# JettHuang/jet-pbrt

Hardware: AMD Instinct MI355X
Metric: Msamples/sec (whole node) + per-pixel L2 vs CPU ref, cornell_box 1024spp (higher is better)
Workload: dtype f32

## Files before the change

jet-pbrt_amd/csrc/jp_device.h:

```cpp
#pragma once
#include <hip/hip_runtime.h>
#include <stdint.h>
#include "jetpbrt_amd.h"
#include "jp_counter_rng.h"

#define JP_BLOCK 256
#define JP_STACK_DEPTH 32

namespace jp
{
struct V3 { float x, y, z; };
__device__ __forceinline__ V3 mk(float x, float y, float z) { V3 v; v.x = x; v.y = y; v.z = z; return v; }
__device__ __forceinline__ V3 operator+(V3 a, V3 b) { return mk(a.x + b.x, a.y + b.y, a.z + b.z); }
__device__ __forceinline__ V3 operator-(V3 a, V3 b) { return mk(a.x - b.x, a.y - b.y, a.z - b.z); }
__device__ __forceinline__ V3 operator-(V3 a) { return mk(-a.x, -a.y, -a.z); }
__device__ __forceinline__ V3 operator*(V3 a, float s) { return mk(a.x * s, a.y * s, a.z * s); }
__device__ __forceinline__ V3 operator*(float s, V3 a) { return mk(a.x * s, a.y * s, a.z * s); }
__device__ __forceinline__ V3 operator/(V3 a, float s) { return mk(a.x / s, a.y / s, a.z / s); }
__device__ __forceinline__ V3 cmul(V3 a, V3 b) { return mk(a.x * b.x, a.y * b.y, a.z * b.z); }
__device__ __forceinline__ V3 cdiv(V3 a, V3 b) { return mk(a.x / b.x, a.y / b.y, a.z / b.z); }
__device__ __forceinline__ V3 splat(float v) { return mk(v, v, v); }
__device__ __forceinline__ V3 csqrt(V3 a) { return mk(sqrtf(a.x), sqrtf(a.y), sqrtf(a.z)); }
__device__ __forceinline__ float dot(V3 a, V3 b) { return a.x * b.x + a.y * b.y + a.z * b.z; }
__device__ __forceinline__ float len2(V3 a) { return a.x * a.x + a.y * a.y + a.z * a.z; }
__device__ __forceinline__ float len(V3 a) { return sqrtf(len2(a)); }
__device__ __forceinline__ V3 normalize(V3 a) { return a / len(a); }
__device__ __forceinline__ V3 cross(V3 a, V3 v) { return mk(a.y * v.z - a.z * v.y, a.z * v.x - a.x * v.z, a.x * v.y - a.y * v.x); }
__device__ __forceinline__ float absdot(V3 a, V3 b) { return fabsf(dot(a, b)); }
__device__ __forceinline__ bool isblack(V3 c) { return c.x == 0.f && c.y == 0.f && c.z == 0.f; }
__device__ __forceinline__ float smin(float a, float b) { return (b < a) ? b : a; }
__device__ __forceinline__ float smax(float a, float b) { return (a < b) ? b : a; }
__device__ __forceinline__ float maxcomp(V3 c) { float m = (c.y < c.z) ? c.z : c.y; return (c.x < m) ? m : c.x; }
__device__ __forceinline__ float clampf(float v, float lo, float hi) { if (v < lo) return lo; else if (v > hi) return hi; else return v; }
__device__ __forceinline__ V3 xyz(float4 v) { return mk(v.x, v.y, v.z); }

#define JP_PI      3.14159274101257324219f
#define JP_INF     __int_as_float(0x7f800000)

struct SceneView
{
	const float4* nodes; int n_nodes;
	const float4* prims; const int4* meta; int n_prims;
	const float4* mats;
	const int* mat_type; int n_mats;
	const float4* lights;
	int n_lights;
	const float4* shade_tab;
	float3 env_sum;
	int n_env;
	float world_radius;
	JpCamera cam;
	const float4* flat; int n_flat;
	const uint4* wide; int n_wide;
	const uint4* q4; int n_q4;
	const float4* refbox; float cert_pad, cert_pad_eye;
};

__device__ __forceinline__ bool tri_hit(V3 p0, V3 p1, V3 p2, V3 n, V3 o, V3 d, float tmin, float& tmax)
{
	const V3 oa = p0 - o;
	const float distance = dot(n, oa) / dot(n, d);
	if (!((distance > tmin) && (distance < tmax))) return false;
	const V3 ob = p1 - o, oc = p2 - o;
	const V3 v0 = cross(oc, ob), v1 = cross(ob, oa), v2 = cross(oa, oc);
	const float v0d = dot(v0, d), v1d = dot(v1, d), v2d = dot(v2, d);
	if (((v0d < 0) && (v1d < 0) && (v2d < 0)) || ((v0d >= 0) && (v1d >= 0) && (v2d >= 0))) { tmax = distance; return true; }
	return false;
}
__device__ __forceinline__ bool rect_hit(V3 p0, V3 p1, V3 p2, V3 p3, V3 n, V3 o, V3 d, float tmin, float& tmax)
{
	const V3 oa = p0 - o;
	const float distance = dot(n, oa) / dot(n, d);
	if (!((distance > tmin) && (distance < tmax))) return false;
	const V3 ob = p1 - o, oc = p2 - o, od = p3 - o;
	const V3 v0 = cross(oc, ob), v1 = cross(ob, oa), v2 = cross(oa, od), v3 = cross(od, oc);
	const float v0d = dot(v0, d), v1d = dot(v1, d), v2d = dot(v2, d), v3d = dot(v3, d);
	if (((v0d < 0) && (v1d < 0) && (v2d < 0) && (v3d < 0)) || ((v0d >= 0) && (v1d >= 0) && (v2d >= 0) && (v3d >= 0))) { tmax = distance; return true; }
	return false;
}
__device__ __forceinline__ bool sph_hit(V3 c, float r, V3 o, V3 d, float tmin, float& tmax)
{
	V3 oc = o - c;
	float a = len2(d);
	float half_b = dot(oc, d);
	float cc = len2(oc) - r * r;
	float disc = half_b * half_b - a * cc;
	if (disc > 0.0f)
	{
		float root = sqrtf(disc);
		float time;
		float root1 = (-half_b - root) / a;
		if (root1 < tmax && root1 > tmin) time = root1;
		else
		{
			float root2 = (-half_b + root) / a;
			if (root2 < tmax && root2 > tmin) time = root2;
			else return false;
		}
		tmax = time;
		return true;
	}
	return false;
}

__device__ __forceinline__ bool disk_hit(V3 c, float r, V3 n, V3 o, V3 d, float tmin, float& tmax)
{
	const float dn = dot(d, n);
	if (fabsf(dn - 0.f) <= 1.1920928955078125e-07f * smax(1.f, smax(fabsf(dn), fabsf(0.f)))) return false;
	const V3 op = c - o;
	const float distance = dot(n, op) / dot(n, d);
	if ((distance > tmin) && (distance < tmax))
	{
		const V3 hp = o + distance * d;
		if (len(c - hp) <= r) { tmax = distance; return true; }
	}
	return false;
}

template <int kS, typename PrimPtr>
__device__ __forceinline__ bool prim_hit(PrimPtr prims, int pi, V3 o, V3 d, float tmin, float& tmax)
{
	const float4 g0 = prims[kS * pi + 0], g1 = prims[kS * pi + 1], g2 = prims[kS * pi + 2], g3 = prims[kS * pi + 3];
	const int type = __float_as_int(g3.w);
	if (type == JP_SHAPE_TRIANGLE) return tri_hit(xyz(g0), xyz(g1), xyz(g2), xyz(g3), o, d, tmin, tmax);
	if (type == JP_SHAPE_SPHERE) return sph_hit(xyz(g0), g0.w, o, d, tmin, tmax);
	if (type == JP_SHAPE_DISK) return disk_hit(xyz(g0), g0.w, xyz(g1), o, d, tmin, tmax);
	return rect_hit(xyz(g0), xyz(g1), xyz(g2), mk(g0.w, g1.w, g2.w), xyz(g3), o, d, tmin, tmax);
}

template <bool kAnyHit, int kS, typename NodePtr, typename PrimPtr>
__device__ __forceinline__ int traverse(NodePtr nodes, PrimPtr prims, V3 o, V3 d, float tmin, float& tmax, int* stack)
{
	const float ix = 1.0f / d.x, iy = 1.0f / d.y, iz = 1.0f / d.z;
	int hit = -1, sp = 0, cur = 0;
	for (;;)
	{
		bool alive = true;
		while (cur >= 0)
		{
			const float4 n0 = nodes[kS * cur + 0], n1 = nodes[kS * cur + 1], n2 = nodes[kS * cur + 2], n3 = nodes[kS * cur + 3];
			const float lx0 = (n0.x - o.x) * ix, lx1 = (n0.w - o.x) * ix;
			const float ly0 = (n0.y - o.y) * iy, ly1 = (n1.x - o.y) * iy;
			const float lz0 = (n0.z - o.z) * iz, lz1 = (n1.y - o.z) * iz;
			const float ln = fmaxf(fmaxf(fminf(lx0, lx1), fminf(ly0, ly1)), fmaxf(fminf(lz0, lz1), tmin));
			const float lf = fminf(fminf(fmaxf(lx0, lx1), fmaxf(ly0, ly1)), fminf(fmaxf(lz0, lz1), tmax));
			const float rx0 = (n1.z - o.x) * ix, rx1 = (n2.y - o.x) * ix;
			const float ry0 = (n1.w - o.y) * iy, ry1 = (n2.z - o.y) * iy;
			const float rz0 = (n2.x - o.z) * iz, rz1 = (n2.w - o.z) * iz;
			const float rn = fmaxf(fmaxf(fminf(rx0, rx1), fminf(ry0, ry1)), fmaxf(fminf(rz0, rz1), tmin));
			const float rf = fminf(fminf(fmaxf(rx0, rx1), fmaxf(ry0, ry1)), fminf(fmaxf(rz0, rz1), tmax));
			const bool hl = ln <= lf * 1.000002f, hr = rn <= rf * 1.000002f;
			const int cl = __float_as_int(n3.x), cr = __float_as_int(n3.y);
			if (hl && hr)
			{
				const bool leftFirst = kAnyHit ? true : (ln <= rn);
				cur = leftFirst ? cl : cr;
				stack[sp * JP_BLOCK] = leftFirst ? cr : cl; sp++;
			}
			else if (hl) cur = cl;
			else if (hr) cur = cr;
			else if (sp > 0) { sp--; cur = stack[sp * JP_BLOCK]; }
			else { alive = false; break; }
		}
		if (!alive) break;
		const int e = -cur - 1, first = e >> 4, count = (e & 15) + 1;
		for (int k = 0; k < count; k++)
			if (prim_hit<kS>(prims, first + k, o, d, tmin, tmax)) { hit = first + k; if (kAnyHit) return hit; }
		if (sp > 0) { sp--; cur = stack[sp * JP_BLOCK]; } else break;
	}
	return hit;
}

__device__ __forceinline__ bool ref_box_exact(float4 n0, float4 n1, V3 o, V3 d, float tmin, float tmax)
{
	float bt0 = tmin, bt1 = tmax;
	{
		const float lo = (n0.x - o.x) / d.x, hi = (n1.x - o.x) / d.x;
		bt0 = smax(smin(lo, hi), bt0); bt1 = smin(smax(lo, hi), bt1);
		if (bt1 <= bt0) return false;
	}
	{
		const float lo = (n0.y - o.y) / d.y, hi = (n1.y - o.y) / d.y;
		bt0 = smax(smin(lo, hi), bt0); bt1 = smin(smax(lo, hi), bt1);
		if (bt1 <= bt0) return false;
	}
	{
		const float lo = (n0.z - o.z) / d.z, hi = (n1.z - o.z) / d.z;
		bt0 = smax(smin(lo, hi), bt0); bt1 = smin(smax(lo, hi), bt1);
		if (bt1 <= bt0) return false;
	}
	return true;
}
__device__ __forceinline__ bool ref_box(float4 n0, float4 n1, V3 o, V3 d, V3 rd, float tmin, float tmax)
{
	const float x0 = (n0.x - o.x) * rd.x, x1 = (n1.x - o.x) * rd.x;
	const float y0 = (n0.y - o.y) * rd.y, y1 = (n1.y - o.y) * rd.y;
	const float z0 = (n0.z - o.z) * rd.z, z1 = (n1.z - o.z) * rd.z;
	const float t0 = fmaxf(fmaxf(fminf(x0, x1), fminf(y0, y1)), fmaxf(fminf(z0, z1), tmin));
	const float t1 = fminf(fminf(fmaxf(x0, x1), fmaxf(y0, y1)), fminf(fmaxf(z0, z1), tmax));
	const float s = x0 + x1 + y0 + y1 + z0 + z1;
	const float margin = 2e-6f * (fabsf(t0) + fabsf(t1));
	const float gap = t1 - t0;
	if (fabsf(s) <= 3.0e38f && fabsf(gap) > margin) return gap > 0.f;
	return ref_box_exact(n0, n1, o, d, tmin, tmax);
}

template <bool kAnyHit>
__device__ __forceinline__ int traverse_ref(const float4* __restrict__ nodes, const float4* __restrict__ prims, V3 o, V3 d, float tmin, float& tmax, int* stack)
{
	const V3 rd = mk(__builtin_amdgcn_rcpf(d.x), __builtin_amdgcn_rcpf(d.y), __builtin_amdgcn_rcpf(d.z));
	int hit = -1, sp = 0, cur = 0;
	for (;;)
	{
		const float4 n0 = nodes[2 * cur], n1 = nodes[2 * cur + 1];
		const bool ok = ref_box(n0, n1, o, d, rd, tmin, tmax);
		const int left = __float_as_int(n0.w), right = __float_as_int(n1.w);
		if (ok && left >= 0) { stack[sp * JP_BLOCK] = right; sp++; cur = left; continue; }
		if (ok)
		{
			const int first = -left - 1;
			for (int k = 0; k < right; k++)
				if (prim_hit<4>(prims, first + k, o, d, tmin, tmax)) { hit = first + k; if (kAnyHit) return hit; }
		}
		if (sp == 0) break;
		sp--; cur = stack[sp * JP_BLOCK];
	}
	return hit;
}

typedef const __attribute__((address_space(4))) float* ConstFPtr;
typedef unsigned long long u64;
template <bool k64> struct FlatMask { typedef unsigned int type; };
template <> struct FlatMask<true> { typedef u64 type; };
template <bool k64> __device__ __forceinline__ int mask_count(typename FlatMask<k64>::type m) { return k64 ? __popcll((u64)m) : __popc((unsigned int)m); }

template <bool k64>
__device__ __forceinline__ typename FlatMask<k64>::type flat_boxes(const float4* flat_g, int n_flat, V3 o, V3 d, float tmin, float tmax)
{
	typedef typename FlatMask<k64>::type M;
	ConstFPtr flat = (ConstFPtr)flat_g;
	const float ix = __builtin_amdgcn_rcpf(d.x), iy = __builtin_amdgcn_rcpf(d.y), iz = __builtin_amdgcn_rcpf(d.z);
	M mask = 0;
	#define JP_FLAT_BOX(i) \
	{ \
		const float x0 = (flat[8 * (i) + 0] - o.x) * ix, x1 = (flat[8 * (i) + 4] - o.x) * ix; \
		const float y0 = (flat[8 * (i) + 1] - o.y) * iy, y1 = (flat[8 * (i) + 5] - o.y) * iy; \
		const float z0 = (flat[8 * (i) + 2] - o.z) * iz, z1 = (flat[8 * (i) + 6] - o.z) * iz; \
		const float tn = fmaxf(fmaxf(fminf(x0, x1), fminf(y0, y1)), fmaxf(fminf(z0, z1), tmin)); \
		const float tf = fminf(fminf(fmaxf(x0, x1), fmaxf(y0, y1)), fminf(fmaxf(z0, z1), tmax)); \
		M bits = (M)__float_as_uint(flat[8 * (i) + 3]); \
		if (k64) bits |= (M)((u64)__float_as_uint(flat[8 * (i) + 7]) << 32); \
		if (tn <= tf * 1.000002f) mask |= bits; \
	}
	int i0 = 0;
	for (; i0 + 4 <= n_flat; i0 += 4)
	{
		#pragma unroll
		for (int u = 0; u < 4; u++) JP_FLAT_BOX(i0 + u)
	}
	for (; i0 < n_flat; i0++) JP_FLAT_BOX(i0)
	#undef JP_FLAT_BOX
	return mask;
}

template <bool kAnyHit, bool k64, int kS, typename PrimPtr>
__device__ __forceinline__ int flat_prims(typename FlatMask<k64>::type mask, PrimPtr prims, V3 o, V3 d, float tmin, float& tmax)
{
	int hit = -1;
#ifdef JP_DBG_FLAT_P1ONLY
	mask = mask == (typename FlatMask<k64>::type)0x12345677u ? 1u : 0u;
#endif
	while (mask)
	{
		const int p = (k64 ? __ffsll((unsigned long long)mask) : __ffs((int)mask)) - 1;
		mask &= mask - 1;
		if (prim_hit<kS>(prims, p, o, d, tmin, tmax)) { hit = p; if (kAnyHit) return hit; }
	}
	return hit;
}

template <bool kAnyHit, int kS, typename PrimPtr>
__device__ __forceinline__ int traverse_flat(const float4* flat_g, int n_flat, int n_prims, PrimPtr prims, V3 o, V3 d, float tmin, float& tmax)
{
	if (n_prims > 32) return flat_prims<kAnyHit, true, kS>(flat_boxes<true>(flat_g, n_flat, o, d, tmin, tmax), prims, o, d, tmin, tmax);
	return flat_prims<kAnyHit, false, kS>(flat_boxes<false>(flat_g, n_flat, o, d, tmin, tmax), prims, o, d, tmin, tmax);
}

template <bool kAnyHit, typename PrimPtr>
__device__ __forceinline__ int traverse_wide(const uint4* __restrict__ wide, PrimPtr prims, V3 o, V3 d, float tmin, float& tmax, unsigned int* stack)
{
	const float ix = 1.0f / d.x, iy = 1.0f / d.y, iz = 1.0f / d.z;
	const unsigned int octinv = 7u - ((d.x < 0 ? 1u : 0u) | (d.y < 0 ? 2u : 0u) | (d.z < 0 ? 4u : 0u));
	unsigned int ngx = 0, ngy = 0x80000000u;
	int hit = -1, sp = 0;
	for (;;)
	{
		unsigned int tgx = 0, tgy = 0;
		if (ngy > 0x00ffffffu)
		{
			const unsigned int bit = 31u - (unsigned int)__clz((int)ngy);
			ngy &= ~(1u << bit);
			if (ngy > 0x00ffffffu) { stack[(2 * sp) * JP_BLOCK] = ngx; stack[(2 * sp + 1) * JP_BLOCK] = ngy; sp++; }
			const unsigned int slot = (bit - 24u) ^ octinv;
			const unsigned int rel = (unsigned int)__popc(ngy & 0xffu & ~(0xffffffffu << slot));
			const unsigned int idx = ngx + rel;
			const uint4 q0 = wide[5 * idx + 0], q1 = wide[5 * idx + 1], q2 = wide[5 * idx + 2], q3 = wide[5 * idx + 3], q4 = wide[5 * idx + 4];
			const float sx = __uint_as_float(((q0.w & 0xffu) ) << 23), sy = __uint_as_float(((q0.w >> 8) & 0xffu) << 23), sz = __uint_as_float(((q0.w >> 16) & 0xffu) << 23);
			const float px = __uint_as_float(q0.x) - o.x, py = __uint_as_float(q0.y) - o.y, pz = __uint_as_float(q0.z) - o.z;
			unsigned int hm = 0;
			#pragma unroll
			for (int i = 0; i < 8; i++)
			{
				const int sh = 8 * (i & 3);
				const unsigned int m = ((i < 4 ? q1.z : q1.w) >> sh) & 0xffu;
				const float lx = (float)(((i < 4 ? q2.x : q2.y) >> sh) & 0xffu), ly = (float)(((i < 4 ? q2.z : q2.w) >> sh) & 0xffu), lz = (float)(((i < 4 ? q3.x : q3.y) >> sh) & 0xffu);
				const float hx = (float)(((i < 4 ? q3.z : q3.w) >> sh) & 0xffu), hy = (float)(((i < 4 ? q4.x : q4.y) >> sh) & 0xffu), hz = (float)(((i < 4 ? q4.z : q4.w) >> sh) & 0xffu);
				const float x0 = fmaf(lx, sx, px) * ix, x1 = fmaf(hx, sx, px) * ix;
				const float y0 = fmaf(ly, sy, py) * iy, y1 = fmaf(hy, sy, py) * iy;
				const float z0 = fmaf(lz, sz, pz) * iz, z1 = fmaf(hz, sz, pz) * iz;
				const float tn = fmaxf(fmaxf(fminf(x0, x1), fminf(y0, y1)), fmaxf(fminf(z0, z1), tmin));
				const float tf = fminf(fminf(fmaxf(x0, x1), fmaxf(y0, y1)), fminf(fmaxf(z0, z1), tmax));
				if (m != 0u && tn <= tf * 1.000002f)
				{
					const bool inner = (m & 0x18u) == 0x18u;
					const unsigned int bits = inner ? 1u : (m >> 5), at = inner ? 24u + ((m & 7u) ^ octinv) : (m & 31u);
					hm |= bits << at;
				}
			}
			ngx = q1.x; ngy = (hm & 0xff000000u) | (q0.w >> 24);
			tgx = q1.y; tgy = hm & 0x00ffffffu;
		}
		while (tgy)
		{
			const int j = __ffs((int)tgy) - 1;
			tgy &= tgy - 1;
			if (prim_hit<4>(prims, (int)tgx + j, o, d, tmin, tmax)) { hit = (int)tgx + j; if (kAnyHit) return hit; }
		}
		if (ngy <= 0x00ffffffu)
		{
			if (sp == 0) break;
			sp--; ngx = stack[(2 * sp) * JP_BLOCK]; ngy = stack[(2 * sp + 1) * JP_BLOCK];
		}
	}
	return hit;
}

struct WalkStack
{
	int* lds; int* spill; int cap; unsigned int stride;
	__device__ __forceinline__ void put(int at, int v) const { if (at < cap) lds[at * JP_BLOCK] = v; else spill[(size_t)(at - cap) * stride] = v; }
	__device__ __forceinline__ int get(int at) const { return at < cap ? lds[at * JP_BLOCK] : spill[(size_t)(at - cap) * stride]; }
};

template <int kMode> struct Walker;

template <> struct Walker<0>
{
	V3 o, d; float ix, iy, iz, tmin, tmax; int cur, sp, hit; bool done;
	__device__ __forceinline__ void start(V3 o_, V3 d_, float tmin_, float tmax_)
	{ o = o_; d = d_; ix = 1.0f / d.x; iy = 1.0f / d.y; iz = 1.0f / d.z; tmin = tmin_; tmax = tmax_; cur = 0; sp = 0; hit = -1; done = false; }
	__device__ __forceinline__ bool heavy() const { return cur < 0; }
	template <bool kAnyHit> __device__ __forceinline__ void step(const SceneView& sc, const WalkStack& stack)
	{
		if (cur >= 0)
		{
			const float4* __restrict__ nodes = sc.nodes;
			const float4 n0 = nodes[4 * cur + 0], n1 = nodes[4 * cur + 1], n2 = nodes[4 * cur + 2], n3 = nodes[4 * cur + 3];
			const float lx0 = (n0.x - o.x) * ix, lx1 = (n0.w - o.x) * ix;
			const float ly0 = (n0.y - o.y) * iy, ly1 = (n1.x - o.y) * iy;
			const float lz0 = (n0.z - o.z) * iz, lz1 = (n1.y - o.z) * iz;
			const float ln = fmaxf(fmaxf(fminf(lx0, lx1), fminf(ly0, ly1)), fmaxf(fminf(lz0, lz1), tmin));
			const float lf = fminf(fminf(fmaxf(lx0, lx1), fmaxf(ly0, ly1)), fminf(fmaxf(lz0, lz1), tmax));
			const float rx0 = (n1.z - o.x) * ix, rx1 = (n2.y - o.x) * ix;
			const float ry0 = (n1.w - o.y) * iy, ry1 = (n2.z - o.y) * iy;
			const float rz0 = (n2.x - o.z) * iz, rz1 = (n2.w - o.z) * iz;
			const float rn = fmaxf(fmaxf(fminf(rx0, rx1), fminf(ry0, ry1)), fmaxf(fminf(rz0, rz1), tmin));
			const float rf = fminf(fminf(fmaxf(rx0, rx1), fmaxf(ry0, ry1)), fminf(fmaxf(rz0, rz1), tmax));
			const bool hl = ln <= lf * 1.000002f, hr = rn <= rf * 1.000002f;
			const int cl = __float_as_int(n3.x), cr = __float_as_int(n3.y);
			if (hl && hr)
			{
				const bool leftFirst = kAnyHit ? true : (ln <= rn);
				cur = leftFirst ? cl : cr;
				stack.put(sp, leftFirst ? cr : cl); sp++;
			}
			else if (hl) cur = cl;
			else if (hr) cur = cr;
			else if (sp > 0) { sp--; cur = stack.get(sp); }
			else done = true;
		}
		else
		{
			const int e = -cur - 1, first = e >> 4, count = (e & 15) + 1;
			for (int k = 0; k < count; k++)
				if (prim_hit<4>(sc.prims, first + k, o, d, tmin, tmax)) { hit = first + k; if (kAnyHit) { done = true; return; } }
			if (sp > 0) { sp--; cur = stack.get(sp); } else done = true;
		}
	}
};

template <> struct Walker<5>
{
	V3 o, d, rd; float tmin, tmax; int cur, sp, hit, lfirst, lcount, lk; bool done;
	__device__ __forceinline__ void start(V3 o_, V3 d_, float tmin_, float tmax_)
	{ o = o_; d = d_; rd = mk(__builtin_amdgcn_rcpf(d.x), __builtin_amdgcn_rcpf(d.y), __builtin_amdgcn_rcpf(d.z)); tmin = tmin_; tmax = tmax_; cur = 0; sp = 0; hit = -1; lcount = 0; lk = 0; lfirst = 0; done = false; }
	__device__ __forceinline__ bool heavy() const { return lcount > 0; }
	template <bool kAnyHit> __device__ __forceinline__ void step(const SceneView& sc, const WalkStack& stack)
	{
		if (lcount > 0)
		{
			if (prim_hit<4>(sc.prims, lfirst + lk, o, d, tmin, tmax)) { hit = lfirst + lk; if (kAnyHit) { done = true; return; } }
			if (++lk < lcount) return;
			lcount = 0; lk = 0;
		}
		else
		{
			const float4* __restrict__ nodes = sc.nodes;
			const float4 n0 = nodes[2 * cur], n1 = nodes[2 * cur + 1];
			const bool ok = ref_box(n0, n1, o, d, rd, tmin, tmax);
			const int left = __float_as_int(n0.w), right = __float_as_int(n1.w);
			if (ok && left >= 0) { stack.put(sp, right); sp++; cur = left; return; }
			if (ok && right > 0) { lfirst = -left - 1; lcount = right; lk = 0; return; }
		}
		if (sp == 0) { done = true; return; }
		sp--; cur = stack.get(sp);
	}
};

template <> struct Walker<3>
{
	V3 o, d; float ix, iy, iz, tmin, tmax; unsigned int ngx, ngy, tgx, tgy, octinv; int sp, hit; bool done;
	__device__ __forceinline__ void start(V3 o_, V3 d_, float tmin_, float tmax_)
	{
		o = o_; d = d_; ix = 1.0f / d.x; iy = 1.0f / d.y; iz = 1.0f / d.z; tmin = tmin_; tmax = tmax_;
		octinv = 7u - ((d.x < 0 ? 1u : 0u) | (d.y < 0 ? 2u : 0u) | (d.z < 0 ? 4u : 0u));
		ngx = 0; ngy = 0x80000000u; tgx = tgy = 0; sp = 0; hit = -1; done = false;
	}
	__device__ __forceinline__ bool heavy() const { return tgy == 0u && ngy > 0x00ffffffu; }
// ... 187 lines not shown
```

jet-pbrt_amd/csrc/jp_kernels.hip:

```cpp
#include "jp_common.h"
#include "jp_tex.h"
#include "jp_xbsdf.h"

#include <cstdio>
#include <cstring>
#include <string>
#include <vector>
#include <algorithm>
#include <cmath>
#include <mutex>
#include <thread>
#include "jp_devmem.h"
#include "jp_lbvh.h"
#include "jp_ploc.h"

__global__ void __launch_bounds__(JP_BLOCK) k_raygen(SceneView sc, Queues q, RenderConst rc, DevCounters* cnt)
{
	const unsigned int total = (unsigned int)rc.npix * rc.sbatch;
	const unsigned int nchunks = (total + JP_BLOCK - 1) / JP_BLOCK;
	const unsigned int G = gridDim.x, b = blockIdx.x;
	if (b == 0 && threadIdx.x == 0) { cnt->n_queue[0] = total; cnt->n_queue[1] = 0; cnt->n_shadow = 0; }
	unsigned int filled = 0;
	const unsigned int K = (nchunks + G - 1) / G, npb = (unsigned int)rc.npix / JP_BLOCK;
	for (unsigned int k = 0, j0 = 0; k < K; k++, j0 += JP_BLOCK)
	{
		unsigned int c;
		if (rc.compact) { const unsigned int qi = b * K + k; if (qi >= nchunks) break; const unsigned int pb = qi / (unsigned int)rc.sbatch, sl = qi - pb * (unsigned int)rc.sbatch; c = sl * npb + pb; }
		else { c = b + k * G; if (c >= nchunks) break; }
		const unsigned int slot = c * JP_BLOCK + threadIdx.x;
		if (slot < total)
		{
			const unsigned int i = b * q.R + j0 + threadIdx.x;
			const int pix = slot % rc.npix, s = rc.s0 + slot / rc.npix;
			int x, y; pixel_of(rc, pix, x, y);
			const uint32_t key = jp_rng_key(rc.seed, (uint32_t)x, (uint32_t)y, (uint32_t)s);
			const float fx = (float)x + rngf(rc, key, 0), fy = (float)y + rngf(rc, key, 1);
			const V3 front = mk(sc.cam.front[0], sc.cam.front[1], sc.cam.front[2]);
			const V3 right = mk(sc.cam.right[0], sc.cam.right[1], sc.cam.right[2]);
			const V3 up = mk(sc.cam.up[0], sc.cam.up[1], sc.cam.up[2]);
			V3 dir = front + right * (fx / sc.cam.res_x - 0.5f) + up * (0.5f - fy / sc.cam.res_y);
			dir = normalize(dir);
			q.ray_o[0][i] = make_float4(sc.cam.pos[0], sc.cam.pos[1], sc.cam.pos[2], __int_as_float((int)slot));
			q.ray_d[0][i] = make_float4(dir.x, dir.y, dir.z, __int_as_float(MK_FLAGS(0, 0, 2)));
			q.beta[0][i] = make_float4(1.f, 1.f, 1.f, __int_as_float((int)key));
			q.lacc[slot] = make_float4(0.f, 0.f, 0.f, 0.f);
		}
		const unsigned int left = total - c * JP_BLOCK;
		filled += left < JP_BLOCK ? left : JP_BLOCK;
	}
	if (threadIdx.x == 0) q.blk_q[0][b] = filled;
}


#if defined(JP_SHADE_TIMING) || defined(JP_TRAV_TIMING)
__device__ unsigned long long g_shade_t[16];
#define JP_TSX(i) do { const unsigned long long t_ = __builtin_amdgcn_s_memtime(); t_acc[i] += t_ - t_last; t_last = t_; } while (0)
#endif
#ifdef JP_SHADE_TIMING
#define JP_TS(i) JP_TSX(i)
#else
#define JP_TS(i) do { } while (0)
#endif
#ifdef JP_TRAV_TIMING
#define JP_TT(i) JP_TSX(i)
#else
#define JP_TT(i) do { } while (0)
#endif
template <int kMode>
struct SceneAccess;
template <> struct SceneAccess<0>
{
	const float4 *nodes, *prims; int* stack; int depth;
	__device__ __forceinline__ SceneAccess(const SceneView& sc, int depth_) : nodes(sc.nodes), prims(sc.prims), stack((int*)s_dyn + threadIdx.x), depth(depth_) {}
	template <bool kAnyHit> __device__ __forceinline__ int trace(const SceneView&, V3 o, V3 d, float tmin, float& tmax) const
	{ return traverse<kAnyHit, 4>(nodes, prims, o, d, tmin, tmax, stack); }
};
template <> struct SceneAccess<1>
{
	float4 *nodes, *prims; int* stack; int depth;
	__device__ __forceinline__ SceneAccess(const SceneView& sc, int depth_) : depth(depth_)
	{
		stack = (int*)s_dyn + threadIdx.x;
		nodes = s_dyn + (depth * JP_BLOCK) / 4;
		prims = nodes + 5 * sc.n_nodes;
		for (int i = threadIdx.x; i < 4 * sc.n_nodes; i += JP_BLOCK) nodes[5 * (i >> 2) + (i & 3)] = sc.nodes[i];
		for (int i = threadIdx.x; i < 4 * sc.n_prims; i += JP_BLOCK) prims[5 * (i >> 2) + (i & 3)] = sc.prims[i];
		__syncthreads();
	}
	template <bool kAnyHit> __device__ __forceinline__ int trace(const SceneView&, V3 o, V3 d, float tmin, float& tmax) const
	{ return traverse<kAnyHit, 5>(nodes, prims, o, d, tmin, tmax, stack); }
};
template <> struct SceneAccess<2>
{
	float4* prims;
	__device__ __forceinline__ SceneAccess(const SceneView& sc, int)
	{
		prims = s_dyn;
		for (int i = threadIdx.x; i < 4 * sc.n_prims; i += JP_BLOCK) prims[5 * (i >> 2) + (i & 3)] = sc.prims[i];
		__syncthreads();
	}
	template <bool kAnyHit> __device__ __forceinline__ int trace(const SceneView& sc, V3 o, V3 d, float tmin, float& tmax) const
	{ return traverse_flat<kAnyHit, 5>(sc.flat, sc.n_flat, sc.n_prims, prims, o, d, tmin, tmax); }
};

template <> struct SceneAccess<3>
{
	const float4* prims; unsigned int* stack;
	__device__ __forceinline__ SceneAccess(const SceneView& sc, int) : prims(sc.prims), stack((unsigned int*)s_dyn + threadIdx.x) {}
	template <bool kAnyHit> __device__ __forceinline__ int trace(const SceneView& sc, V3 o, V3 d, float tmin, float& tmax) const
	{ return traverse_wide<kAnyHit>(sc.wide, prims, o, d, tmin, tmax, stack); }
};

template <> struct SceneAccess<4>
{
	WalkStack stack;
	__device__ __forceinline__ SceneAccess(const SceneView&, int depth) { stack.lds = (int*)s_dyn + threadIdx.x; stack.spill = nullptr; stack.cap = depth - 1; stack.stride = 0; }
	template <bool kAnyHit> __device__ __forceinline__ int trace(const SceneView& sc, V3 o, V3 d, float tmin, float& tmax) const
	{ return walk_ray<4, kAnyHit>(sc, o, d, tmin, tmax, stack); }
};

template <> struct SceneAccess<6>
{
	WalkStack stack;
	__device__ __forceinline__ SceneAccess(const SceneView&, int depth) { stack.lds = (int*)s_dyn + threadIdx.x; stack.spill = nullptr; stack.cap = depth - 1; stack.stride = 0; }
	template <bool kAnyHit> __device__ __forceinline__ int trace(const SceneView& sc, V3 o, V3 d, float tmin, float& tmax) const
	{ return walk_ray<6, kAnyHit>(sc, o, d, tmin, tmax, stack); }
};

template <> struct SceneAccess<5>
{
	const float4 *nodes, *prims; int* stack;
	__device__ __forceinline__ SceneAccess(const SceneView& sc, int) : nodes(sc.nodes), prims(sc.prims), stack((int*)s_dyn + threadIdx.x) {}
	template <bool kAnyHit> __device__ __forceinline__ int trace(const SceneView&, V3 o, V3 d, float tmin, float& tmax) const
	{ return traverse_ref<kAnyHit>(nodes, prims, o, d, tmin, tmax, stack); }
};

template <int kMode>
__global__ void __launch_bounds__(JP_BLOCK) k_extend(SceneView sc, Queues q, int cur, int depth, DevCounters* cnt)
{
	SceneAccess<kMode> acc(sc, depth);
	const unsigned int b = blockIdx.x, n = q.blk_q[cur][b], rbase = b * q.R;
	if (b == 0 && threadIdx.x == 0) { cnt->closest += cnt->n_queue[cur]; cnt->n_queue[cur ^ 1] = 0; cnt->n_shadow = 0; }
	unsigned int h = 0;
	float4 ro = make_float4(0, 0, 0, 0), rd = make_float4(0, 0, 1, 0);
	if (threadIdx.x < n) { ro = q.ray_o[cur][rbase + threadIdx.x]; rd = q.ray_d[cur][rbase + threadIdx.x]; }
	for (unsigned int j = threadIdx.x; j < n; j += JP_BLOCK)
	{
		const unsigned int i = rbase + j;
		const float4 co = ro, cd = rd;
		if (j + JP_BLOCK < n) { ro = q.ray_o[cur][i + JP_BLOCK]; rd = q.ray_d[cur][i + JP_BLOCK]; }
		float tmax = JP_INF;
		const int hit = acc.template trace<false>(sc, xyz(co), xyz(cd), 0.001f, tmax);
		q.hit[i] = make_float2(tmax, __int_as_float(hit));
		h += hit >= 0 ? 1u : 0u;
	}
	for (int off = 32; off > 0; off >>= 1) h += __shfl_down(h, off);
	if ((threadIdx.x & 63) == 0 && h) atomicAdd(&cnt->closest_hit, (unsigned long long)h);
}

#ifndef JP_SHADE_TILE
#define JP_SHADE_TILE 8192
#endif
template <bool kTab, bool kPrims, bool kStage, bool kSort, bool kTex, bool kPick>
__device__ __forceinline__ void shade_body(SceneView sc, Queues q, RenderConst rc, int cur, DevCounters* cnt, const TexView& tv, const PickView& pv)
{
	static_assert(kTab || !kPrims, "k_shade: primitive records in LDS only together with the tables");
	constexpr int kWaves = JP_BLOCK / 64, kMaxSeg = (JP_SHADE_TILE / JP_BLOCK) * kWaves;
	static_assert(JP_SHADE_TILE % JP_BLOCK == 0 && JP_SHADE_TILE <= 65536, "k_shade: tile positions are 16-bit");
	__shared__ unsigned short s_idx[kSort ? JP_SHADE_TILE : 1];
	__shared__ unsigned char s_key[kSort ? JP_SHADE_TILE : 1];
	__shared__ unsigned int s_cnt[kSort ? JP_SHADE_CLASSES * kMaxSeg : 1];
	__shared__ unsigned int s_wsum[kWaves];
	__shared__ unsigned int s_ctr[3];
	const unsigned int lane = threadIdx.x & 63u;
	const int n_tab_l = kPick ? 0 : 2 * sc.n_lights;
	const int n_tab = n_tab_l + 4 * sc.n_mats + (sc.n_mats + 3) / 4, n_tab_all = n_tab + (kPrims ? 8 * sc.n_prims : 0);
	float4* s_lights = s_dyn;
	float4* s_mats = s_lights + n_tab_l;
	int* s_mtype = (int*)(s_mats + 4 * sc.n_mats);
	float4* s_prims = s_dyn + n_tab;
	int4* s_meta = (int4*)(s_prims + 4 * sc.n_prims);
	const float4* s_frames = s_prims + 5 * sc.n_prims;
	float4* s_stage = s_dyn + n_tab_all + threadIdx.x;
	const unsigned int b = blockIdx.x, n = q.blk_q[cur][b];
	const int nxt = cur ^ 1;
#ifdef JP_SHADE_TIMING
	unsigned long long t_acc[10] = { 0, 0, 0, 0, 0, 0, 0, 0, 0, 0 }, t_last = __builtin_amdgcn_s_memtime();
#endif
	if (kTab)
	{
		for (int i = threadIdx.x; i < n_tab_all; i += 2 * JP_BLOCK)
		{
			const bool two = i + JP_BLOCK < n_tab_all;
			const float4 a = sc.shade_tab[i], c2 = two ? sc.shade_tab[i + JP_BLOCK] : a;
			s_dyn[i] = a; if (two) s_dyn[i + JP_BLOCK] = c2;
		}
	}
	if (n == 0) { if (threadIdx.x == 0) { q.blk_q[nxt][b] = 0; q.blk_sh[b] = 0; } return; }
	if (threadIdx.x == 0) { s_ctr[0] = 0; s_ctr[1] = 0; s_ctr[2] = 0; }
	__syncthreads();
	const float4* lights = (kTab && !kPick) ? (const float4*)s_lights : sc.lights;
	const float4* mats = kTab ? (const float4*)s_mats : sc.mats;
	const int* mat_type = kTab ? (const int*)s_mtype : sc.mat_type;
	const float4* prims = kPrims ? (const float4*)s_prims : sc.prims;
	const int4* meta_t = kPrims ? (const int4*)s_meta : sc.meta;
	const unsigned int rbase = b * q.R;
	const unsigned int t0 = 0, count = n;
	JP_TS(0);
	if (kSort)
	{
		constexpr unsigned int seg = kMaxSeg, nctr = JP_SHADE_CLASSES * kMaxSeg;
		const unsigned int tid = threadIdx.x;
		const unsigned int plane = tid & 63u, wave = tid >> 6, npass = (count + JP_BLOCK - 1) / JP_BLOCK;
		const unsigned long long ltm = (1ull << plane) - 1ull;
		#pragma unroll 1
		for (unsigned int r0 = 0; r0 < npass; r0 += 8)
		{
			int pi[8];
			#pragma unroll
			for (int u = 0; u < 8; u++)
			{
				const unsigned int j = (r0 + u) * JP_BLOCK + tid;
				pi[u] = j < count ? __float_as_int(q.hit[rbase + t0 + j].y) : -2;
			}
			#pragma unroll
			for (int u = 0; u < 8; u++)
			{
				const unsigned int r = r0 + u;
				if (r >= npass) break;
				unsigned int key = JP_SHADE_CLASSES;
				if (pi[u] != -2)
				{
					int m = -1; if (pi[u] >= 0) m = meta_t[pi[u]].y;
					key = m >= 0 ? 1u + (unsigned int)mat_type[m] : 0u;
				}
				s_key[r * JP_BLOCK + tid] = (unsigned char)key;
				unsigned int mine = 0;
				#pragma unroll
				for (int c = 0; c < JP_SHADE_CLASSES; c++)
				{
					unsigned int nc = 0;
					if ((rc.class_mask >> c) & 1) nc = (unsigned int)__popcll(__ballot(key == (unsigned int)c));
					if (plane == (unsigned int)c) mine = nc;
				}
				if (plane < JP_SHADE_CLASSES) s_cnt[plane * seg + r * kWaves + wave] = mine;
			}
		}
		__syncthreads();
		{
			static_assert(JP_SHADE_CLASSES * kMaxSeg <= 3 * JP_BLOCK, "k_shade: three counters per thread");
			unsigned int v[3], t = 0;
			#pragma unroll
			for (int i = 0; i < 3; i++)
			{
				const unsigned int at = 3 * tid + i;
				v[i] = (at < nctr && (at % seg) / kWaves < npass) ? s_cnt[at] : 0u; t += v[i];
			}
			unsigned int incl = t;
			#pragma unroll
			for (int off = 1; off < 64; off <<= 1) { const unsigned int o = __shfl_up(incl, off); if (plane >= (unsigned int)off) incl += o; }
			if (plane == 63) s_wsum[wave] = incl;
			__syncthreads();
			unsigned int base = incl - t;
			#pragma unroll
			for (int w = 0; w < kWaves; w++) if ((unsigned int)w < wave) base += s_wsum[w];
			#pragma unroll
			for (int i = 0; i < 3; i++) { const unsigned int at = 3 * tid + i; if (at < nctr) s_cnt[at] = base; base += v[i]; }
		}
		__syncthreads();
		#pragma unroll 1
		for (unsigned int r = 0; r < npass; r++)
		{
			const unsigned int key = s_key[r * JP_BLOCK + tid];
			unsigned int pre = 0;
			#pragma unroll
			for (int c = 0; c < JP_SHADE_CLASSES; c++)
			{
				if (!((rc.class_mask >> c) & 1)) continue;
				const unsigned long long m = __ballot(key == (unsigned int)c);
				if (key == (unsigned int)c) pre = (unsigned int)__popcll(m & ltm);
			}
			if (key < JP_SHADE_CLASSES) s_idx[s_cnt[key * seg + r * kWaves + wave] + pre] = (unsigned short)(r * JP_BLOCK + tid);
		}
		__syncthreads();
	}
	float4 ro_n = make_float4(0, 0, 0, 0), rd_n = ro_n, rb_n = ro_n; float2 h_n = make_float2(0, 0); unsigned int s_n = 0;
	JP_TS(1);
	const unsigned int nch = (count + 63u) >> 6;
	unsigned int tk = wave_take(&s_ctr[0], 1u);
	unsigned int c0 = (nch - 1u - tk) << 6;
	if (tk < nch && c0 + lane < count) { const unsigned int pos = c0 + lane, i0 = rbase + t0 + (kSort ? (unsigned int)s_idx[pos] : pos); ro_n = q.ray_o[cur][i0]; rd_n = q.ray_d[cur][i0]; rb_n = q.beta[cur][i0]; h_n = q.hit[i0]; if (kTex) s_n = tv.side[i0]; }
	while (tk < nch)
	{
		const bool valid = c0 + lane < count;
#ifdef JP_SHADE_TIMING
		JP_TS(2);
		asm volatile("s_waitcnt vmcnt(0)" ::: "memory");
		JP_TS(3);
#endif
#ifdef JP_SHADE_NO_PREFETCH
		if (valid) { const unsigned int pos = c0 + lane, i0 = rbase + t0 + (kSort ? (unsigned int)s_idx[pos] : pos); ro_n = q.ray_o[cur][i0]; rd_n = q.ray_d[cur][i0]; rb_n = q.beta[cur][i0]; h_n = q.hit[i0]; if (kTex) s_n = tv.side[i0]; }
		const float4 ro = ro_n, rd = rd_n, rb = rb_n; const float2 h = h_n; const unsigned int sw = s_n;
		tk = wave_take(&s_ctr[0], 1u); c0 = (nch - 1u - tk) << 6;
#else
		const float4 ro = ro_n, rd = rd_n, rb = rb_n; const float2 h = h_n; const unsigned int sw = s_n;
		tk = wave_take(&s_ctr[0], 1u); c0 = (nch - 1u - tk) << 6;
		if (tk < nch && c0 + lane < count)
		{
			const unsigned int pos = c0 + lane;
			const unsigned int i1 = rbase + t0 + (kSort ? (unsigned int)s_idx[pos] : pos);
			ro_n = q.ray_o[cur][i1]; rd_n = q.ray_d[cur][i1]; rb_n = q.beta[cur][i1]; h_n = q.hit[i1]; if (kTex) s_n = tv.side[i1];
		}
#endif
		bool shaded = false, wantNee = false, alive = false;
		V3 o = mk(0, 0, 0), d = mk(0, 0, 1), beta = mk(0, 0, 0), p = mk(0, 0, 0), N = mk(0, 0, 1);
		int slot = 0, bounce = 0; bool spec = false; unsigned int dim = 0; uint32_t key = 0;
		Closure c; c.kind = CL_LAMBERT; Frame fr; fr.s = fr.t = fr.n = mk(0, 0, 1);
		if (valid)
		{
			o = xyz(ro); d = xyz(rd); beta = xyz(rb);
			slot = __float_as_int(ro.w); key = (uint32_t)__float_as_int(rb.w);
			const int flags = __float_as_int(rd.w);
			bounce = FLAG_BOUNCE(flags); spec = FLAG_SPEC(flags); dim = FLAG_DIM(flags);
			const int pi = __float_as_int(h.y);
			const bool found = pi >= 0;
			int mat = -1, hitprim = 0; bool nflip = false, tabframe = kPrims;
			V3 Le = splat(0);
			if (found)
			{
				const float4 g3 = prims[4 * pi + 3];
				const int4 meta = meta_t[pi];
				const int type = __float_as_int(g3.w);
				p = o + h.x * d;
				if (type == JP_SHAPE_TRIANGLE) N = xyz(g3);
				else if (type == JP_SHAPE_RECTANGLE) { nflip = !(dot(xyz(g3), d) <= 0); N = nflip ? -xyz(g3) : xyz(g3); }
				else if (type == JP_SHAPE_DISK) N = xyz(prims[4 * pi + 1]);
				else { const float4 g0 = prims[4 * pi]; N = normalize(p - xyz(g0)); tabframe = false; }
				hitprim = pi;
				mat = meta.y;
				if (meta.z >= 0 && (bounce == 0 || spec))
				{
					const V3 wo = -d;
					if (dot(N, wo) > 0.f) Le = xyz(lights[2 * meta.z]);
				}
			}
			else if (bounce == 0 || spec)
			{
				if (kPick)
				{
					for (int e = 0; e < pv.n_env; e++)
					{
						float4 L = q.lacc[slot];
						V3 a = mk(L.x, L.y, L.z) + cmul(beta, xyz(pv.env[e]));
						q.lacc[slot] = make_float4(a.x, a.y, a.z, 0.f);
					}
				}
				else for (int li = 0; li < sc.n_lights; li++)
				{
					const float4 l0 = lights[2 * li];
					if (__float_as_int(l0.w) == JP_LIGHT_ENVIRONMENT && !isblack(xyz(l0)))
					{
						float4 L = q.lacc[slot];
						V3 a = mk(L.x, L.y, L.z) + cmul(beta, xyz(l0));
						q.lacc[slot] = make_float4(a.x, a.y, a.z, 0.f);
					}
				}
			}
			if (!isblack(Le))
			{
				float4 L = q.lacc[slot];
				V3 a = mk(L.x, L.y, L.z) + cmul(beta, Le);
				q.lacc[slot] = make_float4(a.x, a.y, a.z, 0.f);
			}
			if (found && bounce < rc.max_depth)
			{
				if (mat < 0) alive = true;
				else
				{
					float up = 0.f;
					const int mtype = mat_type[mat];
					if (mtype == JP_MAT_PLASTIC) up = rngf(rc, key, dim++);
					if (kTex && sw != 0u) make_closure_tex(mats, mtype, mat, up, tex_color(tv, sw), c);
					else make_closure(mats, mtype, mat, up, c);
#ifdef JP_DBG_SKIP_FRAME
					fr.n = N; fr.s = mk(N.y, N.z, N.x); fr.t = mk(N.z, N.x, N.y);
#else
					if (kPrims && tabframe)
					{
						const float4 fn = s_frames[3 * hitprim], fs = s_frames[3 * hitprim + 1], ft = s_frames[3 * hitprim + 2];
						fr.n = nflip ? -xyz(fn) : xyz(fn); fr.s = xyz(fs); fr.t = nflip ? -xyz(ft) : xyz(ft);
					}
					else fr = frame_from_z(N);
#endif
					shaded = true;
					wantNee = !is_delta(c);
#ifdef JP_DBG_SKIP_NEE
					wantNee = false;
#endif
				}
			}
		}
		JP_TS(4);
		unsigned int qs = 0;
		if (!kStage)
		{
			const unsigned long long mn = __ballot(wantNee);
			if (mn) qs = rbase + wave_take(&s_ctr[2], (unsigned int)__popcll(mn)) + (unsigned int)__popcll(mn & ((1ull << lane) - 1ull));
		}
		V3 nd = d, nbeta = beta; int nbounce = bounce; bool nspec = spec;
		V3 wo = mk(0, 0, 1);
		int k = 0;
		if (shaded)
		{
			const V3 wo_w = -d;
			wo = to_local(fr, wo_w);
			closure_set_wo(c, wo);
			if (wantNee)
			{
				const int nl = kPick ? (sc.n_lights > 0 ? 1 : 0) : sc.n_lights;
				for (int it = 0; it < nl; it++)
				{
					int li = it; float pmf = 1.f;
					if (kPick)
					{
						const float u0 = rngf(rc, key, dim), u1 = rngf(rc, key, dim + 1); dim += 2;
						li = light_pick(pv, u0, u1, pmf);
					}
					const unsigned int d0 = dim; dim += 2;
					if (kPick && !(pmf > 0.f)) continue;
					const float4 lrad = lights[2 * li];
					if (isblack(xyz(lrad))) continue;
					const float ux = rngf(rc, key, d0), uy = rngf(rc, key, d0 + 1);
					LightSample ls = sample_li(sc, prims, lights, li, p, N, ux, uy);
					if (isblack(ls.Li) || ls.pdf == 0.f) continue;
					const V3 f = eval_local(c, wo, to_local(fr, ls.wi));
					if (isblack(f)) continue;
					const V3 sdir = __float_as_int(lrad.w) == JP_LIGHT_AREA ? ls.wi : normalize(ls.pos - p);
					const float dist = ls.dist >= 0.f ? ls.dist : len(p - ls.pos);
					V3 contrib = cmul(cmul(beta, f), ls.Li) * absdot(ls.wi, N) / ls.pdf;
					if (kPick) contrib = contrib / pmf;
					if (k < rc.n_planes)
					{
						if (kStage)
						{
							s_stage[(2 * k) * JP_BLOCK] = make_float4(sdir.x, sdir.y, sdir.z, dist - 0.001f);
							s_stage[(2 * k + 1) * JP_BLOCK] = make_float4(contrib.x, contrib.y, contrib.z, 0.f);
						}
						else
						{
							q.sh_d[(size_t)k * q.cap + qs] = make_float4(sdir.x, sdir.y, sdir.z, dist - 0.001f);
							q.sh_c[(size_t)k * q.cap + qs] = make_float4(contrib.x, contrib.y, contrib.z, 0.f);
						}
						k++;
					}
				}
				if (!kStage) q.sh_o[qs] = make_float4(p.x, p.y, p.z, __int_as_float(slot | (k << rc.slot_bits)));
			}
		}
		JP_TS(5);
#ifdef JP_DBG_SKIP_SAMPLE
		if (false)
#else
		if (shaded)
#endif
		{
			const float ux = rngf(rc, key, dim), uy = rngf(rc, key, dim + 1); dim += 2;
			BsdfSample bs = sample_local(c, wo, ux, uy);
			bs.wi = to_world(fr, bs.wi);
			if (!(isblack(bs.f) || bs.pdf == 0.f))
			{
				nspec = (bs.flags & BS_SPECULAR) != 0;
				if (bounce >= 3)
				{
					const float qq = smax(0.05f, 1 - maxcomp(bs.f));
					const float ur = rngf(rc, key, dim++);
					if (!(ur < qq))
					{
						nbeta = cmul(beta, bs.f * absdot(bs.wi, N) / (bs.pdf * (1 - qq)));
						alive = true;
					}
				}
				else
				{
					nbeta = cmul(beta, bs.f * absdot(bs.wi, N) / bs.pdf);
					alive = true;
				}
				nd = bs.wi; nbounce = bounce + 1;
			}
		}
		JP_TS(6);
		unsigned int j = 0;
		const unsigned long long lt = (1ull << lane) - 1ull;
		const unsigned long long ma = __ballot(alive);
		if (kStage)
		{
			const unsigned long long ms = __ballot(k > 0);
			if (ma | ms)
			{
				const unsigned int base = wave_take(&s_ctr[1], (unsigned int)__popcll(ma) | ((unsigned int)__popcll(ms) << 16));
				j = rbase + (base & 0xffffu) + (unsigned int)__popcll(ma & lt);
				qs = rbase + (base >> 16) + (unsigned int)__popcll(ms & lt);
			}
			if (k > 0)
			{
				q.sh_o[qs] = make_float4(p.x, p.y, p.z, __int_as_float(slot | (k << rc.slot_bits)));
				for (int kk = 0; kk < k; kk++)
				{
					q.sh_d[(size_t)kk * q.cap + qs] = s_stage[(2 * kk) * JP_BLOCK];
					q.sh_c[(size_t)kk * q.cap + qs] = s_stage[(2 * kk + 1) * JP_BLOCK];
				}
			}
		}
		else if (ma) j = rbase + wave_take(&s_ctr[1], (unsigned int)__popcll(ma)) + (unsigned int)__popcll(ma & lt);
		if (alive)
		{
			q.ray_o[nxt][j] = make_float4(p.x, p.y, p.z, __int_as_float(slot));
			q.ray_d[nxt][j] = make_float4(nd.x, nd.y, nd.z, __int_as_float(MK_FLAGS(nbounce, nspec, dim)));
			q.beta[nxt][j] = make_float4(nbeta.x, nbeta.y, nbeta.z, __int_as_float((int)key));
		}
		JP_TS(7);
#ifdef JP_SHADE_TIMING
		asm volatile("s_waitcnt vmcnt(0)" ::: "memory");
		JP_TS(9);
#endif
	}
	JP_TS(2);
	__syncthreads();
	JP_TS(8);
#ifdef JP_SHADE_TIMING
	if (lane == 0) for (int i = 0; i < 10; i++) atomicAdd(&g_shade_t[i], t_acc[i]);
	if (lane == 0) atomicAdd(&g_shade_t[15], 1ull);
#endif
	if (threadIdx.x == 0)
	{
		const unsigned int run_q = kStage ? (s_ctr[1] & 0xffffu) : s_ctr[1], run_sh = kStage ? (s_ctr[1] >> 16) : s_ctr[2];
		q.blk_q[nxt][b] = run_q; q.blk_sh[b] = run_sh;
		if (run_q) atomicAdd(&cnt->n_queue[nxt], run_q);
		if (run_sh) atomicAdd(&cnt->n_shadow, run_sh);
	}
}
template <bool kTab, bool kPrims, bool kStage, bool kSort>
__global__ void __launch_bounds__(JP_BLOCK) k_shade(SceneView sc, Queues q, RenderConst rc, int cur, DevCounters* cnt)
{
	const TexView tv = {}; const PickView pv = {};
	shade_body<kTab, kPrims, kStage, kSort, false, false>(sc, q, rc, cur, cnt, tv, pv);
}

template <int kMode>
__global__ void __launch_bounds__(JP_BLOCK, 4) k_shadow(SceneView sc, Queues q, RenderConst rc, int depth, DevCounters* cnt)
{
#ifdef JP_TRAV_TIMING
	unsigned long long t_acc[10] = { 0, 0, 0, 0, 0, 0, 0, 0, 0, 0 }, t_last = __builtin_amdgcn_s_memtime();
#endif
	SceneAccess<kMode> acc(sc, depth);
	const unsigned int b = blockIdx.x, E = q.blk_sh[b], rbase = b * q.R;
	JP_TT(0);
	unsigned int rays = 0, occ = 0;
	float4 so_n = make_float4(0, 0, 0, 0), sd_n = make_float4(0, 0, 1, 0);
	if (threadIdx.x < E) { so_n = q.sh_o[rbase + threadIdx.x]; sd_n = q.sh_d[rbase + threadIdx.x]; }
	for (unsigned int j = threadIdx.x; j < E; j += JP_BLOCK)
	{
		const unsigned int e = rbase + j;
#ifdef JP_TRAV_TIMING
		JP_TT(1);
		asm volatile("s_waitcnt vmcnt(0)" ::: "memory");
		JP_TT(2);
#endif
		const float4 so = so_n; float4 sd = sd_n;
		if (j + JP_BLOCK < E) { so_n = q.sh_o[e + JP_BLOCK]; sd_n = q.sh_d[e + JP_BLOCK]; }
		const int packed = __float_as_int(so.w);
		const int slot = packed & ((1 << rc.slot_bits) - 1), n = (int)((unsigned int)packed >> rc.slot_bits);
		if (n == 0) continue;
		bool any = false;
		const float4 L = q.lacc[slot];
		V3 a = mk(L.x, L.y, L.z);
		for (int k = 0; k < n; k++)
		{
			const float4 c4 = q.sh_c[(size_t)k * q.cap + e];
			float tmax = sd.w;
			const V3 dir = xyz(sd);
			if (k + 1 < n) sd = q.sh_d[(size_t)(k + 1) * q.cap + e];
			JP_TT(3);
#ifdef JP_TRAV_TIMING
			int hit;
			if constexpr (kMode == 2)
			{
				const unsigned int m = flat_boxes<false>(sc.flat, sc.n_flat, xyz(so), dir, 0.001f, tmax);
				JP_TT(4);
				hit = flat_prims<true, false, 5>(m, acc.prims, xyz(so), dir, 0.001f, tmax);
				JP_TT(5);
			}
			else hit = acc.template trace<true>(sc, xyz(so), dir, 0.001f, tmax);
#else
			const int hit = acc.template trace<true>(sc, xyz(so), dir, 0.001f, tmax);
#endif
			rays++;
			if (hit >= 0) occ++;
			else { a = a + xyz(c4); any = true; }
			JP_TT(6);
		}
		if (any) q.lacc[slot] = make_float4(a.x, a.y, a.z, 0.f);
		JP_TT(7);
	}
#ifdef JP_TRAV_TIMING
	JP_TT(1);
	if ((threadIdx.x & 63) == 0) { for (int i = 0; i < 8; i++) atomicAdd(&g_shade_t[i], t_acc[i]); atomicAdd(&g_shade_t[15], 1ull); }
#endif
	for (int off = 32; off > 0; off >>= 1) { rays += __shfl_down(rays, off); occ += __shfl_down(occ, off); }
	if ((threadIdx.x & 63) == 0) { if (rays) atomicAdd(&cnt->shadow, (unsigned long long)rays); if (occ) atomicAdd(&cnt->shadow_occ, (unsigned long long)occ); }
}

template <int kMode, bool kAnyHit, bool kVote>
__device__ __forceinline__ void persist_turn(Walker<kMode>& w, const SceneView& sc, const WalkStack& stack, bool pool)
{
	const int nh = __popcll(__ballot(!w.done && w.heavy())), nl = __popcll(__ballot(!w.done && !w.heavy()));
	const bool heavyTurn = kVote ? nh > nl : w.heavy();
	if (kVote) { JP_TURN(heavyTurn ? 3 : 0, 1); JP_TURN(heavyTurn ? 4 : 1, heavyTurn ? nh : nl); JP_TURN(heavyTurn ? 5 : 2, nh + nl); if (!pool) { JP_TURN(8, 1); JP_TURN(9, nh + nl); JP_TURN(10, heavyTurn ? nh : nl); } }
	if (!w.done && (w.heavy() == heavyTurn)) w.template step<kAnyHit>(sc, stack);
}
__device__ __forceinline__ unsigned int lane_rank(unsigned long long m) { return __builtin_amdgcn_mbcnt_hi((unsigned int)(m >> 32), __builtin_amdgcn_mbcnt_lo((unsigned int)m, 0u)); }

#ifndef JP_CERT_WAVES
#define JP_CERT_WAVES 8
#endif
template <int kMode, int kRefill, bool kVote>
__global__ void __launch_bounds__(JP_BLOCK, (kMode == 6 ? JP_CERT_WAVES : 8)) k_extend_persist(SceneView sc, Queues q, int cur_q, int stack_cap, int* spill, DevCounters* cnt)
{
	__shared__ unsigned int s_next;
	const WalkStack stack = { (int*)s_dyn + threadIdx.x, spill + blockIdx.x * JP_BLOCK + threadIdx.x, (kMode == 4 || kMode == 6) ? stack_cap - 1 : stack_cap, gridDim.x * JP_BLOCK };
	const unsigned int b = blockIdx.x, n = q.blk_q[cur_q][b], rbase = b * q.R;
	if (b == 0 && threadIdx.x == 0) { cnt->closest += cnt->n_queue[cur_q]; cnt->n_queue[cur_q ^ 1] = 0; cnt->n_shadow = 0; }
	if (threadIdx.x == 0) s_next = 0;
	__syncthreads();
	const int lane = threadIdx.x & 63;
	Walker<kMode> w; w.done = true; w.hit = -1; w.tmax = JP_INF;
	unsigned int ridx = 0xffffffffu, h = 0;
	bool pool = n > 0;
	for (;;)
	{
		const unsigned long long idle = __ballot(w.done);
		const int nidle = __popcll(idle);
		if (nidle == 64 || (pool && nidle >= kRefill))
		{
			if (w.done && ridx != 0xffffffffu)
			{
				int hp = w.hit;
				if constexpr (kMode == 6) { if (!w.certain(sc)) hp = -2; }
				q.hit[rbase + ridx] = make_float2(w.tmax, __int_as_float(hp)); h += hp >= 0 ? 1u : 0u; ridx = 0xffffffffu;
			}
			if (!pool) break;
			const int first = __ffsll((long long)idle) - 1;
			unsigned int start = 0;
			if (lane == first) start = atomicAdd(&s_next, (unsigned int)nidle);
			start = __shfl(start, first);
			{ constexpr bool kAnyHit = false; (void)kAnyHit; JP_TURN(6, 1); JP_TURN(7, nidle); }
			pool = start + (unsigned int)nidle < n;
			if (w.done)
			{
				const unsigned int my = start + lane_rank(idle);
				if (my < n)
				{
					const float4 ro = q.ray_o[cur_q][rbase + my], rd = q.ray_d[cur_q][rbase + my];
					w.start(xyz(ro), xyz(rd), 0.001f, JP_INF);
					if constexpr (kMode == 6) w.mark_origin(sc);
					ridx = my;
				}
			}
			if (start >= n && nidle == 64) break;
			continue;
		}
		persist_turn<kMode, false, kVote>(w, sc, stack, pool);
	}
	if constexpr (kMode == 6)
	{
		__syncthreads();
		for (unsigned int i = threadIdx.x; i < n; i += JP_BLOCK)
		{
			if (__float_as_int(q.hit[rbase + i].y) != -2) continue;
			const float4 ro = q.ray_o[cur_q][rbase + i], rd = q.ray_d[cur_q][rbase + i];
			float tm = JP_INF;
			const int hp = walk_ray<5, false>(sc, xyz(ro), xyz(rd), 0.001f, tm, stack);
			q.hit[rbase + i] = make_float2(tm, __int_as_float(hp)); h += hp >= 0 ? 1u : 0u;
			if (cnt) atomicAdd(&cnt->cert_fallback, 1ull);
		}
	}
	for (int off = 32; off > 0; off >>= 1) h += __shfl_down(h, off);
	if (lane == 0 && h) atomicAdd(&cnt->closest_hit, (unsigned long long)h);
}

template <int kMode, int kRefill, bool kVote>
__global__ void __launch_bounds__(JP_BLOCK, (kMode == 6 ? JP_CERT_WAVES : 8)) k_shadow_persist(SceneView sc, Queues q, RenderConst rc, int stack_cap, int* spill, DevCounters* cnt)
{
	__shared__ unsigned int s_next;
	const WalkStack stack = { (int*)s_dyn + threadIdx.x, spill + blockIdx.x * JP_BLOCK + threadIdx.x, (kMode == 4 || kMode == 6) ? stack_cap - 1 : stack_cap, gridDim.x * JP_BLOCK };
	unsigned int* s_occ = (unsigned int*)s_dyn + stack_cap * JP_BLOCK;
	const unsigned int b = blockIdx.x, E = q.blk_sh[b], rbase = b * q.R;
	const unsigned int NP = (unsigned int)rc.n_planes, total = E * NP;
	unsigned int* s_uns = s_occ + ((size_t)q.R * NP + 31) / 32;
	for (unsigned int i = threadIdx.x; i < (total + 31) / 32; i += JP_BLOCK) { s_occ[i] = 0; if (kMode == 6) s_uns[i] = 0; }
	if (threadIdx.x == 0) s_next = 0;
	__syncthreads();
	const int lane = threadIdx.x & 63;
	Walker<kMode> w; w.done = true; w.hit = -1;
	unsigned int rid = 0xffffffffu;
	bool pool = total > 0;
	for (;;)
	{
		const unsigned long long idle = __ballot(w.done);
		const int nidle = __popcll(idle);
		if (nidle == 64 || (pool && nidle >= kRefill))
		{
			if (w.done && rid != 0xffffffffu)
			{
				if (w.hit >= 0) atomicOr(&s_occ[rid >> 5], 1u << (rid & 31u));
				if constexpr (kMode == 6) { if (w.hit < 0 && w.unsure) atomicOr(&s_uns[rid >> 5], 1u << (rid & 31u)); }
				rid = 0xffffffffu;
			}
			if (!pool) break;
			const int first = __ffsll((long long)idle) - 1;
			unsigned int start = 0;
			if (lane == first) start = atomicAdd(&s_next, (unsigned int)nidle);
			start = __shfl(start, first);
			{ constexpr bool kAnyHit = true; (void)kAnyHit; JP_TURN(6, 1); JP_TURN(7, nidle); }
			pool = start + (unsigned int)nidle < total;
			if (w.done)
			{
				const unsigned int my = start + lane_rank(idle);
				if (my < total)
				{
					const unsigned int k = my / E, e = my - k * E;
					const float4 so = q.sh_o[rbase + e];
					if (k < ((unsigned int)__float_as_int(so.w) >> rc.slot_bits))
					{
						const float4 sd = q.sh_d[(size_t)k * q.cap + rbase + e];
						w.start(xyz(so), xyz(sd), 0.001f, sd.w);
						rid = my;
					}
				}
			}
			if (start >= total && nidle == 64) break;
			continue;
		}
// ... 336 lines not shown
```

jet-pbrt_amd/csrc/jp_render.h:

```cpp
#pragma once
namespace
{
enum { CLS_EXTEND = 0, CLS_SHADE = 1, CLS_SHADOW = 2, CLS_OTHER = 3, CLS_PATH = 4 };

void free_queues(JpContext* c) { c->qb = QueueBufs(); c->cap = 0; c->planes_alloc = 0; c->blk_alloc = 0; }

int ensure_queues(JpContext* c, unsigned int cap, int planes, unsigned int nblocks)
{
	if (c->cap >= cap && c->planes_alloc >= planes && c->blk_alloc >= nblocks) return JP_OK;
	cap = std::max(cap, c->cap); planes = std::max(planes, c->planes_alloc); nblocks = std::max(nblocks, c->blk_alloc);
	free_queues(c);
	auto alloc = [](DevBuf& b, auto*& p, size_t bytes) { return reserve(b, p, bytes) == hipSuccess; };
	Queues& q = c->q; QueueBufs& qb = c->qb; bool ok = true;
	for (int b = 0; b < 2 && ok; b++) ok = alloc(qb.ray_o[b], q.ray_o[b], (size_t)cap * 16) && alloc(qb.ray_d[b], q.ray_d[b], (size_t)cap * 16) && alloc(qb.beta[b], q.beta[b], (size_t)cap * 16)
	                                       && alloc(qb.blk_q[b], q.blk_q[b], (size_t)nblocks * 4);
	ok = ok && alloc(qb.hit, q.hit, (size_t)cap * 8) && alloc(qb.lacc, q.lacc, (size_t)cap * 16) && alloc(qb.sh_o, q.sh_o, (size_t)cap * 16)
	     && alloc(qb.sh_d, q.sh_d, (size_t)cap * 16 * planes) && alloc(qb.sh_c, q.sh_c, (size_t)cap * 16 * planes) && alloc(qb.blk_sh, q.blk_sh, (size_t)nblocks * 4);
	if (!ok) { free_queues(c); return fail(JP_ERR_DEVICE, "jp_render: out of device memory for the path queues"); }
	c->cap = cap; c->planes_alloc = planes; c->blk_alloc = nblocks;
	return JP_OK;
}

int ensure_gamma(JpContext* c)
{
	if (!c->gamma) HIP_TRY(upload(c->gamma, host_gamma_thresholds(), 255 * sizeof(float)));
	return JP_OK;
}
int ensure_rgb8(JpContext* c, size_t n)
{
	if (const int e = reserve_idle(c, c->rgb8, n); e != JP_OK) return e;
	return ensure_gamma(c);
}
void tonemap8(JpContext* c, const float* src, size_t n)
{
	hipLaunchKernelGGL(k_tonemap8, dim3((unsigned int)std::min<size_t>((size_t)c->n_cus * 8, (n + JP_BLOCK - 1) / JP_BLOCK)), dim3(JP_BLOCK), 0, c->stream, src, c->rgb8.get<unsigned char>(), c->gamma.get<const float>(), n);
}

struct Stamper
{
	JpContext* c; int cls; size_t a;
	Stamper(JpContext* c, int cls) : c(c), cls(cls), a(0)
	{
		if (!c->profiling) return;
		if (c->evused + 2 > c->evpool.size()) { size_t old = c->evpool.size(); c->evpool.resize(old + 64); for (size_t i = old; i < c->evpool.size(); i++) hipEventCreate(&c->evpool[i]); }
		a = c->evused; c->evused += 2;
		hipEventRecord(c->evpool[a], c->stream);
	}
	~Stamper() { if (!c->profiling) return; hipEventRecord(c->evpool[a + 1], c->stream); JpContext::Stamp s = { cls, a, a + 1 }; c->stamps.push_back(s); }
};

struct Shard { int band, count, index, local_rows, lane_rows; };
int shard_of(const JpRenderParams* rp, Shard& s, int lane_index = 0, int lane_count = 1, int lane_group = 4)
{
	if (rp->width <= 0 || rp->height <= 0 || rp->spp <= 0 || rp->max_depth < 0 || rp->max_depth > 200) return fail(JP_ERR_INVALID_ARGUMENT, "jp_render: bad width/height/spp/max_depth");
	if (rp->integrator < JP_INTEGRATOR_PATH || rp->integrator > JP_INTEGRATOR_DEBUG_NORMAL) return fail(JP_ERR_INVALID_ARGUMENT, "jp_render: unknown integrator");
	if (rp->integrator == JP_INTEGRATOR_WHITTED && rp->max_depth > JP_WHITTED_MAX_DEPTH) return fail(JP_ERR_UNSUPPORTED, "jp_render: the Whitted integrator supports max_depth <= 16");
	if (rp->sampler_mode != JP_SAMPLER_COUNTER && rp->sampler_mode != JP_SAMPLER_DEBUG) return fail(JP_ERR_UNSUPPORTED, "jp_render: the device path implements the counter sampler only (the sequential mt19937_64 stream is not reproducible in parallel)");
	s.band = rp->band_rows > 0 ? rp->band_rows : 20;
	s.count = rp->shard_count > 1 ? rp->shard_count : 1;
	s.index = s.count > 1 ? rp->shard_index : 0;
	if (s.index < 0 || s.index >= s.count) return fail(JP_ERR_INVALID_ARGUMENT, "jp_render: shard_index out of range");
	const int nbands = (rp->height + s.band - 1) / s.band;
	s.local_rows = 0;
	for (int b = s.index; b < nbands; b += s.count) s.local_rows += std::min(s.band, rp->height - b * s.band);
	s.lane_rows = 0;
	for (int g0 = lane_index * lane_group; g0 < s.local_rows; g0 += lane_count * lane_group) s.lane_rows += std::min(lane_group, s.local_rows - g0);
	return JP_OK;
}

inline bool refill_walks(const ScenePlan& p) { return p.persist && (p.trav_mode == 0 || p.trav_mode == 3 || p.trav_mode == 5); }
inline int refill_row(const ScenePlan& p) { return p.persist >= 32 ? 2 : (p.persist >= 16 ? 1 : 0); }
inline int extend_depth(const ScenePlan& p) { return (p.trav_mode == 5 ? p.cert : p.use_q4) ? p.stack_depth_q4 : p.stack_depth; }
inline int shadow_depth(const ScenePlan& p) { return (p.trav_mode == 5 ? p.cert : p.q4_shadow) ? p.stack_depth_q4 : (p.trav_mode == 3 ? (int)(p.lds_bytes_shadow / (JP_BLOCK * sizeof(int))) : p.stack_depth); }
inline int deepest_walk(const ScenePlan& p) { return std::max(std::max(p.stack_depth, p.stack_depth_q4), p.trav_mode == 3 ? (int)(p.lds_bytes_shadow / (JP_BLOCK * sizeof(int))) : 0); }
inline size_t spill_need(const ScenePlan& p, int deep, unsigned int G) { return deep >= p.stack_lds_words ? (size_t)(deep - p.stack_lds_words + 1) * G * JP_BLOCK : 1; }

typedef void (*ExtendKernel)(SceneView, Queues, int, int, DevCounters*);
typedef void (*ExtendRefillKernel)(SceneView, Queues, int, int, int*, DevCounters*);
struct ExtendLaunch { ExtendRefillKernel refill; ExtendKernel plain; size_t lds; int words; };
template <int M> ExtendRefillKernel extend_refill(const ScenePlan& p)
{
	static const ExtendRefillKernel k[3][2] = { { k_extend_persist<M, 8, false>, k_extend_persist<M, 8, true> }, { k_extend_persist<M, 16, false>, k_extend_persist<M, 16, true> }, { k_extend_persist<M, 32, false>, k_extend_persist<M, 32, true> } };
	return k[refill_row(p)][p.vote];
}
ExtendLaunch extend_kernel(const ScenePlan& p)
{
	if (!refill_walks(p)) return { nullptr, p.trav_mode == 5 ? k_extend<5> : (p.trav_mode == 2 ? k_extend<2> : (p.trav_mode == 1 ? k_extend<1> : k_extend<0>)), p.lds_bytes, p.stack_depth };
	const int words = std::min(extend_depth(p), p.stack_lds_words);
	const ExtendRefillKernel k = p.trav_mode == 5 ? (p.cert ? extend_refill<6>(p) : extend_refill<5>(p)) : (p.use_q4 ? extend_refill<4>(p) : extend_refill<0>(p));
	return { k, nullptr, (size_t)words * JP_BLOCK * sizeof(int), words };
}

typedef void (*ShadowKernel)(SceneView, Queues, RenderConst, int, DevCounters*);
typedef void (*ShadowRefillKernel)(SceneView, Queues, RenderConst, int, int*, DevCounters*);
struct ShadowLaunch { ShadowRefillKernel refill; ShadowKernel plain; size_t lds; int words; bool cert_fell_back; };
template <int M> ShadowRefillKernel shadow_refill(const ScenePlan& p)
{
	static const ShadowRefillKernel k[3][2] = { { k_shadow_persist<M, 8, false>, k_shadow_persist<M, 8, true> }, { k_shadow_persist<M, 16, false>, k_shadow_persist<M, 16, true> }, { k_shadow_persist<M, 32, false>, k_shadow_persist<M, 32, true> } };
	return k[refill_row(p)][p.vote];
}
ShadowLaunch shadow_kernel(const ScenePlan& p, unsigned int R)
{
	const int words = std::min(shadow_depth(p), p.stack_lds_words);
	const size_t plds = (size_t)words * JP_BLOCK * sizeof(int) + (((size_t)R * p.n_planes + 31) / 32) * 4 * (p.cert ? 2 : 1);
	if (!refill_walks(p) || plds > 64 * 1024)
		return { nullptr, p.trav_mode == 3 ? k_shadow<3> : (p.trav_mode == 5 ? k_shadow<5> : (p.trav_mode == 2 ? k_shadow<2> : (p.trav_mode == 1 ? k_shadow<1> : k_shadow<0>))), p.trav_mode == 3 ? p.lds_bytes_shadow : p.lds_bytes, p.stack_depth, p.cert };
	const ShadowRefillKernel k = p.trav_mode == 5 ? (p.cert ? shadow_refill<6>(p) : shadow_refill<5>(p)) : (p.q4_shadow ? shadow_refill<4>(p) : (p.trav_mode == 3 ? shadow_refill<3>(p) : shadow_refill<0>(p)));
	return { k, nullptr, plds, words, false };
}

typedef void (*ShadeKernel)(SceneView, Queues, RenderConst, int, DevCounters*);
typedef void (*ShadeTexKernel)(SceneView, Queues, RenderConst, int, DevCounters*, TexView);
struct ShadeKernels { ShadeKernel plain; ShadeTexKernel tex; };
template <bool kTab, bool kPrims, bool kStage> ShadeKernels shade_row(bool sort)
{
	ShadeKernels k = { sort ? k_shade<kTab, kPrims, kStage, true> : k_shade<kTab, kPrims, kStage, false>, sort ? k_shade_tex<kTab, kPrims, kStage, true> : k_shade_tex<kTab, kPrims, kStage, false> };
	return k;
}
ShadeKernels shade_kernels(const ScenePlan& p)
{
	if (p.shade_prims_in_lds) return p.stage_nee ? shade_row<true, true, true>(p.shade_sort) : shade_row<true, true, false>(p.shade_sort);
	if (p.tables_in_lds) return p.stage_nee ? shade_row<true, false, true>(p.shade_sort) : shade_row<true, false, false>(p.shade_sort);
	return shade_row<false, false, false>(p.shade_sort);
}

typedef void (*ShadePickKernel)(SceneView, Queues, RenderConst, int, DevCounters*, PickView);
typedef void (*ShadePickTexKernel)(SceneView, Queues, RenderConst, int, DevCounters*, TexView, PickView);
struct ShadePickKernels { ShadePickKernel plain; ShadePickTexKernel tex; };
ShadePickKernels shade_pick_kernels(const ScenePlan& p);

typedef void (*OtherKernel)(SceneView, Queues, RenderConst, int, int, DevCounters*);
OtherKernel other_kernel(const ScenePlan& p) { return p.trav_mode == 5 ? k_other<5> : (p.trav_mode == 2 ? k_other<2> : (p.trav_mode == 1 ? k_other<1> : k_other<0>)); }

typedef void (*TraceKernel)(SceneView, int, int, const float*, const float*, const float*, const float*, int*, float*, int*, float*);
typedef void (*SurfaceKernel)(SceneView, TexView, int, int, const float*, const float*, const float*, const float*, int*, float*, float*);
struct TraceLaunch { TraceKernel trace; SurfaceKernel surface; size_t lds; int depth; };
template <int M> TraceLaunch trace_row(size_t lds, int depth) { TraceLaunch t = { k_trace<M>, k_surface<M>, lds, depth }; return t; }
TraceLaunch trace_kernel(const ScenePlan& p, int tw)
{
	const size_t q4lds = (size_t)p.stack_depth_q4 * JP_BLOCK * sizeof(int);
	if (p.trav_mode == 3 && tw == 2) { TraceLaunch t = { k_trace<3>, nullptr, p.lds_bytes_shadow, p.stack_depth }; return t; }
	if (p.trav_mode == 5 && p.cert && q4lds <= 64 * 1024 && tw != 3) return trace_row<6>(q4lds, p.stack_depth_q4);
	if (p.trav_mode == 5) return trace_row<5>(p.lds_bytes, p.stack_depth);
	if (p.use_q4 && q4lds <= 64 * 1024 && tw != 1) return trace_row<4>(q4lds, p.stack_depth_q4);
	return p.trav_mode == 2 ? trace_row<2>(p.lds_bytes, p.stack_depth) : (p.trav_mode == 1 ? trace_row<1>(p.lds_bytes, p.stack_depth) : trace_row<0>(p.lds_bytes, p.stack_depth));
}

int render_one(JpContext* c, const JpRenderParams* rp, float* film_dev, bool sync, int lane_index = 0, int lane_count = 1, int lane_group = 4, bool ev0_recorded = false)
{
	if (!c->plan.have_scene) return fail(JP_ERR_NO_SCENE, "jp_render: no scene uploaded");
	const ScenePlan& p = c->plan; Shard sh; DevCounters* const d_cnt = c->cnt.get<DevCounters>();
	if (const int e = shard_of(rp, sh, lane_index, lane_count, lane_group); e != JP_OK) return e;
	HIP_TRY(hipSetDevice(c->device));
	const long long npix = (long long)sh.lane_rows * rp->width;

	if (!ev0_recorded) HIP_TRY(hipEventRecord(c->ev0, c->stream));
	HIP_TRY(hipMemsetAsync(film_dev, 0, sizeof(float) * 3 * (size_t)rp->width * rp->height, c->stream));
	HIP_TRY(hipMemsetAsync(d_cnt, 0, sizeof(DevCounters), c->stream));
	c->evused = 0; c->stamps.clear();
	unsigned long long samples = 0;
	if (npix > 0)
	{
		if (npix > (1 << 24)) return fail(JP_ERR_UNSUPPORTED, "jp_render: more than 2^24 pixels per shard");
		const int slot_bits = p.n_planes <= 31 ? 27 : 24;
		const unsigned int PMAX = slot_bits == 27 ? (1u << 26) : (1u << 24);
		size_t freeB = 0, totalB = 0; hipMemGetInfo(&freeB, &totalB);
		const size_t per = 136 + 32 * (size_t)p.n_planes;
		size_t budget = std::min<size_t>((size_t)24 << 30, (freeB / (size_t)std::max(1, lane_count) + (c->cap ? (size_t)c->cap * (136 + 32 * (size_t)c->planes_alloc) : 0)) / 2);
		if (c->opt.max_slots > 0) budget = std::min<size_t>(budget, (size_t)c->opt.max_slots * per);
		int sbatch = 1; unsigned int P = 0, G = 1, R = JP_BLOCK, cap = 0;
		for (int attempt = 0;; attempt++)
		{
			const unsigned int pcap = (unsigned int)std::min<size_t>(PMAX, std::max<size_t>((size_t)npix, budget / per));
			sbatch = (int)std::max<long long>(1, std::min<long long>(rp->spp, pcap / npix));
			{
				const int nb = (rp->spp + sbatch - 1) / sbatch;
				sbatch = (rp->spp + nb - 1) / nb;
			}
			if ((long long)sbatch * npix > (long long)PMAX) return fail(JP_ERR_UNSUPPORTED, "jp_render: shard too large for one batch");
			P = (unsigned int)((long long)sbatch * npix);
			const unsigned int nchunks = (P + JP_BLOCK - 1) / JP_BLOCK;
			G = std::max(1u, std::min(nchunks, (unsigned int)(c->n_cus * c->blocks_per_cu)));
			G = std::max(G, (nchunks + JP_SHADE_TILE / JP_BLOCK - 1) / (JP_SHADE_TILE / JP_BLOCK));
			R = ((nchunks + G - 1) / G) * JP_BLOCK;
			cap = G * R;
			const int st = ensure_queues(c, cap, p.n_planes, G);
			if (st == JP_OK) break;
			if (sbatch <= 1 || attempt >= 6) return st;
			budget = (size_t)sbatch / 2 * (size_t)npix * per;
		}
		c->q.cap = cap; c->q.R = R;
		const bool tex = p.textured && rp->integrator == JP_INTEGRATOR_PATH;
		if (tex) if (const int e = reserve_idle(c, c->side, (size_t)cap * sizeof(unsigned int)); e != JP_OK) return e;
		TexView tv = p.tv; tv.side = c->side.get<unsigned int>();
		if (const int e = reserve_idle(c, c->spill, spill_need(p, p.persist ? deepest_walk(p) : 0, G) * sizeof(int)); e != JP_OK) return e;
		if (const int e = reserve_idle(c, c->pix_acc, (size_t)npix * 16); e != JP_OK) return e;
		int* const d_spill = c->spill.get<int>(); float4* const d_pix_acc = c->pix_acc.get<float4>();

		RenderConst rc; rc.width = rp->width; rc.height = rp->height; rc.spp = rp->spp; rc.max_depth = rp->max_depth; rc.seed = rp->seed;
		rc.band_rows = sh.band; rc.shard_index = sh.index; rc.shard_count = sh.count; rc.npix = (int)npix; rc.local_rows = sh.lane_rows; rc.n_planes = p.n_planes;
		rc.lane_index = lane_index; rc.lane_count = lane_count; rc.lane_rows = lane_group; rc.class_mask = p.class_mask; rc.sampler_debug = rp->sampler_mode == JP_SAMPLER_DEBUG ? 1 : 0;
		rc.slot_bits = slot_bits;
		rc.tiled = 0;
		rc.compact = (p.trav_mode != 2 && p.trav_mode != 1 && npix % JP_BLOCK == 0) ? 1 : 0;
		if (c->opt.compact_regions != 0) rc.compact = (c->opt.compact_regions > 0 && npix % JP_BLOCK == 0) ? 1 : 0;
		const int grid = (int)G;
		const ExtendLaunch ek = extend_kernel(p); const ShadowLaunch sk = shadow_kernel(p, R); const ShadeKernels hk = shade_kernels(p); const OtherKernel ok = other_kernel(p);
		const ShadePickKernels pk = p.pick ? shade_pick_kernels(p) : ShadePickKernels{ nullptr, nullptr };
		for (int s0 = 0; s0 < rp->spp; s0 += sbatch)
		{
			rc.s0 = s0; rc.sbatch = std::min(sbatch, rp->spp - s0);
			{ Stamper t(c, CLS_OTHER); hipLaunchKernelGGL(k_raygen, dim3(grid), dim3(JP_BLOCK), 0, c->stream, p.sv, c->q, rc, d_cnt); }
			if (rp->integrator != JP_INTEGRATOR_PATH)
			{
				Stamper t(c, CLS_OTHER);
				const int ogrid = (int)std::min<unsigned int>((P + JP_BLOCK - 1) / JP_BLOCK, (unsigned int)(c->n_cus * 16));
				hipLaunchKernelGGL(ok, dim3(ogrid), dim3(JP_BLOCK), p.lds_bytes, c->stream, p.sv, c->q, rc, rp->integrator, p.stack_depth, d_cnt);
			}
			int cur = 0;
			int iters = rp->integrator != JP_INTEGRATOR_PATH ? 0 : rp->max_depth + 1;
			for (int it = 0;; it++)
			{
				if (it >= iters)
				{
					if (rp->integrator != JP_INTEGRATOR_PATH || !p.has_null_material || it > iters + 64) break;
					DevCounters h; HIP_TRY(hipMemcpyAsync(&h, d_cnt, sizeof(h), hipMemcpyDeviceToHost, c->stream)); HIP_TRY(hipStreamSynchronize(c->stream));
					if (h.n_queue[cur] == 0) break;
				}
				{
					Stamper t(c, CLS_EXTEND);
					if (ek.refill) hipLaunchKernelGGL(ek.refill, dim3(grid), dim3(JP_BLOCK), ek.lds, c->stream, p.sv, c->q, cur, ek.words, d_spill, d_cnt);
					else hipLaunchKernelGGL(ek.plain, dim3(grid), dim3(JP_BLOCK), ek.lds, c->stream, p.sv, c->q, cur, ek.words, d_cnt);
				}
				{
					Stamper t(c, CLS_SHADE);
					if (tex)
					{
						hipLaunchKernelGGL(k_texel, dim3(grid), dim3(JP_BLOCK), 0, c->stream, p.sv, c->q, cur, tv);
						if (p.pick) hipLaunchKernelGGL(pk.tex, dim3(grid), dim3(JP_BLOCK), p.shade_lds_bytes, c->stream, p.sv, c->q, rc, cur, d_cnt, tv, p.pv);
						else hipLaunchKernelGGL(hk.tex, dim3(grid), dim3(JP_BLOCK), p.shade_lds_bytes, c->stream, p.sv, c->q, rc, cur, d_cnt, tv);
					}
					else if (p.pick) hipLaunchKernelGGL(pk.plain, dim3(grid), dim3(JP_BLOCK), p.shade_lds_bytes, c->stream, p.sv, c->q, rc, cur, d_cnt, p.pv);
					else hipLaunchKernelGGL(hk.plain, dim3(grid), dim3(JP_BLOCK), p.shade_lds_bytes, c->stream, p.sv, c->q, rc, cur, d_cnt);
				}
				HIP_TRY(hipGetLastError());
				if (it < rp->max_depth || p.has_null_material)
				{
					Stamper t(c, CLS_SHADOW);
					if (sk.cert_fell_back) c->cert_fell_back = true;
					if (sk.refill) hipLaunchKernelGGL(sk.refill, dim3(grid), dim3(JP_BLOCK), sk.lds, c->stream, p.sv, c->q, rc, sk.words, d_spill, d_cnt);
					else hipLaunchKernelGGL(sk.plain, dim3(grid), dim3(JP_BLOCK), sk.lds, c->stream, p.sv, c->q, rc, sk.words, d_cnt);
					HIP_TRY(hipGetLastError());
				}
				cur ^= 1;
			}
			{ Stamper t(c, CLS_OTHER); hipLaunchKernelGGL(k_resolve, dim3((unsigned int)std::min<long long>(c->n_cus * 8, (npix + JP_BLOCK - 1) / JP_BLOCK)), dim3(JP_BLOCK), 0, c->stream, c->q, rc, d_pix_acc, film_dev, s0 == 0 ? 1 : 0, s0 + rc.sbatch >= rp->spp ? 1 : 0); }
			samples += (unsigned long long)rc.sbatch * (unsigned long long)npix;
		}
		HIP_TRY(hipGetLastError());
	}
	HIP_TRY(hipEventRecord(c->ev1, c->stream));
	c->own_samples = samples;
	if (sync) HIP_TRY(hipStreamSynchronize(c->stream));
	return JP_OK;
}

__global__ void __launch_bounds__(JP_BLOCK) k_add_film(float* __restrict__ dst, const float* __restrict__ src, size_t n)
{
	for (size_t i = (size_t)blockIdx.x * JP_BLOCK + threadIdx.x; i < n; i += (size_t)gridDim.x * JP_BLOCK) dst[i] += src[i];
}

int make_lanes(JpContext* c, int extra)
{
	if (!c->ev_added && hipEventCreateWithFlags(&c->ev_added, hipEventDisableTiming) != hipSuccess) return fail(JP_ERR_DEVICE, "jp_render: event allocation failed");
	while ((int)c->lanes.size() < extra)
	{
		JpContext* l = new JpContext;
		l->device = c->device; l->is_lane = true; l->n_cus = c->n_cus; l->blocks_per_cu = c->blocks_per_cu; l->opt = c->opt; l->opt_env = c->opt_env;
		std::memset(&l->counters, 0, sizeof(l->counters)); std::memset(&l->q, 0, sizeof(l->q));
		if (hipStreamCreateWithFlags(&l->stream, hipStreamNonBlocking) != hipSuccess || hipEventCreate(&l->ev0) != hipSuccess || hipEventCreate(&l->ev1) != hipSuccess
		    || l->cnt.reserve(sizeof(DevCounters)) != hipSuccess)
		{ jp_destroy_context(l); return fail(JP_ERR_DEVICE, "jp_render: stream/event allocation for an extra lane failed"); }
		c->lanes.push_back(l);
	}
	return JP_OK;
}

void sync_lane_scene(JpContext* c, JpContext* l)
{
	l->plan = c->plan;
	if (!l->plan.textured && l->side) { hipStreamSynchronize(l->stream); l->side.reset(); }
	l->profiling = c->profiling; l->opt = c->opt;
}

bool fused_eligible(const JpContext* c, const JpRenderParams* rp)
{
	if (c->opt.fused <= 0) return false;
	if (c->is_lane || !c->plan.have_scene || rp->integrator != JP_INTEGRATOR_PATH) return false;
	if (!c->plan.tables_in_lds || c->plan.n_planes > 4) return false;
	if (c->plan.cert) return false;
	if (c->plan.textured) return false;
	if (c->plan.pick) return false;
	if (c->plan.trav_mode == 2) return c->plan.shade_prims_in_lds;
	return c->plan.trav_mode == 0 || c->plan.trav_mode == 3 || c->plan.trav_mode == 5;
}

typedef void (*PathKernel)(SceneView, Queues, RenderConst, PathConst, int*, DevCounters*);
PathKernel path_kernel(const ScenePlan& p)
{
	const bool so = p.shade_sort;
	switch (p.trav_mode)
	{
	case 2: return so ? k_path<2, 2, true, true, true> : k_path<2, 2, true, false, true>;
	case 3:
		if (p.use_q4) return p.q4_shadow ? (so ? k_path<4, 4, false, true, true> : k_path<4, 4, false, false, true>) : (so ? k_path<4, 3, false, true, true> : k_path<4, 3, false, false, true>);
		return so ? k_path<0, 3, false, true, true> : k_path<0, 3, false, false, true>;
	case 5: return so ? k_path<5, 5, false, true, false> : k_path<5, 5, false, false, false>;
	default:
		if (p.use_q4) return so ? k_path<4, 4, false, true, true> : k_path<4, 4, false, false, true>;
		return so ? k_path<0, 0, false, true, true> : k_path<0, 0, false, false, true>;
	}
}

int render_fused(JpContext* c, const JpRenderParams* rp, float* film_dev, bool sync)
{
	const ScenePlan& p = c->plan; Shard sh; DevCounters* const d_cnt = c->cnt.get<DevCounters>();
	if (const int e = shard_of(rp, sh); e != JP_OK) return e;
	HIP_TRY(hipSetDevice(c->device));
	const long long npix = (long long)sh.local_rows * rp->width;

	HIP_TRY(hipEventRecord(c->ev0, c->stream));
	HIP_TRY(hipMemsetAsync(film_dev, 0, sizeof(float) * 3 * (size_t)rp->width * rp->height, c->stream));
	HIP_TRY(hipMemsetAsync(d_cnt, 0, sizeof(DevCounters), c->stream));
	c->evused = 0; c->stamps.clear();
	unsigned long long samples = 0;
	c->last_fused = 1; c->last_lanes = 1;
	if (npix > 0)
	{
		if (npix > (1 << 24)) return fail(JP_ERR_UNSUPPORTED, "jp_render: more than 2^24 pixels per shard");
		const PathKernel kern = path_kernel(p);
		const bool flat = p.trav_mode == 2;
		const int modeE = flat ? 2 : (p.trav_mode == 5 ? 5 : 0);
		size_t freeB = 0, totalB = 0; hipMemGetInfo(&freeB, &totalB);
		size_t budget = std::min<size_t>((size_t)4 << 30, (freeB + c->fqb.lacc.bytes()) / 4);
		if (c->opt.max_slots > 0) budget = std::min<size_t>(budget, (size_t)c->opt.max_slots * 16);
		const size_t PMAX = (size_t)1 << 26;
		const size_t pcap = std::min<size_t>(PMAX, std::max<size_t>((size_t)npix, budget / 16));
		int sbatch = (int)std::max<long long>(1, std::min<long long>(rp->spp, (long long)(pcap / (size_t)npix)));
		{ const int nb = (rp->spp + sbatch - 1) / sbatch; sbatch = (rp->spp + nb - 1) / nb; }
		unsigned int R = 1024;
		{ const int v = c->opt.fused_region; if (v >= JP_BLOCK && v <= 8192) R = (unsigned int)(v / JP_BLOCK) * JP_BLOCK; }
		int S = 16;
		{ const int v = c->opt.fused_job_spp; if (v >= 1 && v <= 128) S = v; }
		const int n_tab = 2 * p.sv.n_lights + 4 * p.sv.n_mats + (p.sv.n_mats + 3) / 4, n_tab_all = n_tab + (flat ? 8 * p.sv.n_prims : 0);
		const int deepE = extend_depth(p), deepS = shadow_depth(p);
		const int ecap = flat ? 0 : std::min(deepE, p.stack_lds_words), scap = flat ? 0 : std::min(deepS, p.stack_lds_words);
		PathLds L = path_lds_layout(modeE, n_tab_all, p.sv.n_prims, R, p.n_planes, ecap, scap, p.shade_sort);
		while (L.total > 64 * 1024 && R > JP_BLOCK) { R -= JP_BLOCK; L = path_lds_layout(modeE, n_tab_all, p.sv.n_prims, R, p.n_planes, ecap, scap, p.shade_sort); }
		if (L.total > 64 * 1024) return fail(JP_ERR_UNSUPPORTED, "jp_render: the fused schedule's LDS layout does not fit this scene (JETPBRT_FUSED=0 selects the per-bounce launches)");
		S = std::max(1, std::min(S, std::min(sbatch, (int)(R / 64))));
// ... 336 lines not shown
```

jet-pbrt_amd/csrc/jp_runtime.h:

```cpp
#pragma once

static thread_local std::string g_err;
static int fail(int code, const std::string& msg) { g_err = msg; return code; }
#define HIP_TRY(expr) do { hipError_t _e = (expr); if (_e != hipSuccess) return fail(JP_ERR_DEVICE, std::string(#expr) + ": " + hipGetErrorString(_e)); } while (0)

static inline bool opt_flag(int v, bool dflt) { return v == 0 ? dflt : v > 0; }

static void options_from_environment(JpOptions& o)
{
	struct Item { const char* name; int kind; void* field; int as; };
	const Item items[] = {
		{ "JETPBRT_LANES", 0, &o.lanes, 0 }, { "JETPBRT_LANE_ROWS", 0, &o.lane_rows, 0 }, { "JETPBRT_BLOCKS_PER_CU", 0, &o.blocks_per_cu, 0 }, { "JETPBRT_MAX_SLOTS", 3, &o.max_slots, 0 },
		{ "JETPBRT_COMPACT_REGIONS", 1, &o.compact_regions, 0 }, { "JETPBRT_FUSED", 1, &o.fused, 0 }, { "JETPBRT_REGION", 0, &o.fused_region, 0 }, { "JETPBRT_JOB_SPP", 0, &o.fused_job_spp, 0 },
		{ "JETPBRT_FUSED_WGS", 0, &o.fused_workgroups, 0 }, { "JETPBRT_TRAVERSAL", 6, &o.traversal, 0 }, { "JETPBRT_Q4", 1, &o.q4, 0 }, { "JETPBRT_Q4_SHADOW", 1, &o.q4_shadow, 0 },
		{ "JETPBRT_PERSIST", 2, &o.persist, 0 }, { "JETPBRT_VOTE", 1, &o.vote, 0 }, { "JETPBRT_STACK_LDS", 0, &o.stack_lds_words, 0 }, { "JETPBRT_SHADE_SORT", 1, &o.shade_sort, 0 },
		{ "JETPBRT_DEVICE_TREE", 4, &o.device_tree, 0 }, { "JETPBRT_DEVICE_WIDE", 1, &o.device_wide, 0 }, { "JETPBRT_BVH_MAXLEAF", 0, &o.bvh_max_leaf, 0 },
		{ "JETPBRT_PLOC_RADIUS", 0, &o.ploc_radius, 0 }, { "JETPBRT_PLOC_MAX_ROUNDS", 0, &o.ploc_max_rounds, 0 }, { "JETPBRT_CERTIFIED", 1, &o.certified, 0 },
		{ "JETPBRT_CERT_SLACK", 7, &o.cert_slack, 0 }, { "JETPBRT_CERT_SLACK_EYE", 7, &o.cert_slack_eye, 0 }, { "JETPBRT_CERT_EYE", 7, &o.cert_eye_tau, 0 },
		{ "JETPBRT_SINCOSF", 2, &o.libm_sincosf, 0 }, { "JETPBRT_LIBM", 2, &o.libm_xbsdf, 0 },
		{ "JETPBRT_TRACE_BINARY", 5, &o.trace_walk, 1 }, { "JETPBRT_TRACE_WIDE", 5, &o.trace_walk, 2 }, { "JETPBRT_TRACE_VERBATIM", 5, &o.trace_walk, 3 }, { "JETPBRT_BOX_PAD", 7, &o.box_pad, 0 },
	};
	for (const Item& it : items)
	{
		const char* e = getenv(it.name);
		if (!e || !*e) continue;
		switch (it.kind)
		{
			case 0: *(int32_t*)it.field = atoi(e); break;
			case 1: *(int32_t*)it.field = atoi(e) != 0 ? 1 : -1; break;
			case 2: { const int v = atoi(e); *(int32_t*)it.field = v != 0 ? v : -1; break; }
			case 3: *(int64_t*)it.field = atoll(e); break;
			case 4: *(int32_t*)it.field = std::string(e) == "lbvh" ? 2 : 1; break;
			case 5: *(int32_t*)it.field = it.as; break;
			case 6: { const int v = atoi(e); if (v >= 0 && v <= 3) *(int32_t*)it.field = 1 + v; break; }
			case 7: { const float v = (float)atof(e); *(float*)it.field = v != 0.f ? v : -1.f; break; }
		}
	}
}

struct ScenePlan
{
	bool have_scene = false;
	SceneView sv; TexView tv = {}; bool textured = false;
	PickView pv = {}; bool pick = false;
	int trav_mode = 0, stack_depth = 1, stack_depth_q4 = 0; bool scene_in_lds = false, shade_prims_in_lds = false; size_t lds_bytes = 0, lds_bytes_shadow = 0;
	bool cert = false;
	bool use_q4 = false, q4_shadow = false;
	bool vote = false; int persist = 0;
	int n_planes = 1; bool has_null_material = false;
	bool tables_in_lds = false, stage_nee = false; size_t shade_lds_bytes = 0;
	int class_mask = 0x3f; bool shade_sort = false;
	int stack_lds_words = 12;
};

struct SceneTables
{
	DevBuf nodes, prims, meta, mats, mat_type, lights, shade_tab, flat, wide, q4, refbox;
	DevBuf tex_desc, tex_col, texels, mat_tex, prim_uv;
	DevBuf pick_bins, pick_pmf, pick_env;
};
struct QueueBufs { DevBuf ray_o[2], ray_d[2], beta[2], blk_q[2], hit, lacc, sh_o, sh_d, sh_c, blk_sh; };

struct JpContext
{
	int device = 0;
	JpOptions opt{}, opt_env{};
	hipStream_t stream = nullptr;
	int n_cus = 256;
	ScenePlan plan; SceneTables tab;
	bool cert_fell_back = false; int cert_eye_leaves = 0;
	int sincosf_mode = 0, libm_mode = 0;
	bool build_on_device = false; float build_ms = 0.f; int bvh_height = 0, bvh_nodes = 0;
	Queues q = {}; QueueBufs qb; unsigned int cap = 0; int planes_alloc = 0; unsigned int blk_alloc = 0; int blocks_per_cu = 16;
	DevBuf pix_acc, spill, film;
	DevBuf bsdf_in, bsdf_out, bsdf_fl;
	DevBuf gamma, rgb8; PinnedBuf h_rgb8;
	PinnedBuf h_film;
	DevBuf cnt;
	hipEvent_t ev0 = nullptr, ev1 = nullptr;
	bool profiling = false;
	std::vector<hipEvent_t> evpool; size_t evused = 0;
	struct Stamp { int cls; size_t a, b; };
	std::vector<Stamp> stamps;
	JpCounters counters;
	std::vector<JpContext*> lanes; bool is_lane = false; unsigned long long own_samples = 0; bool bpc_from_env = false;
	hipEvent_t ev_added = nullptr; bool added_valid = false; int last_lanes = 1;
	Queues fq = {}; QueueBufs fqb; unsigned int fcap = 0; int fplanes = 0;
	DevBuf jobs;
	int last_fused = 0, last_region = 0, last_wgs = 0;
	int n_textures = 0, n_tex_mats = 0; long long texel_bytes = 0; int last_textured = 0;
	DevBuf side;
	DevBuf dn_cz[2], dn_nr, dn_stage;
	hipEvent_t dn_ev[2] = { nullptr, nullptr }, gd_ev[2] = { nullptr, nullptr }; bool dn_timed = false, gd_timed = false;
	int last_dn = 0, last_dn_demod = 0, last_guide_spp = 0; float last_dn_sigma[3] = { 0.f, 0.f, 0.f };
	int light_mode = JP_LIGHTS_ALL;
	int n_selectable = 0; double total_weight = 0.0; int last_picked = 0;
};
static int upload_light_table(JpContext* c, const JpScene* s, const std::vector<float>& area);

static int reserve_idle(JpContext* c, DevBuf& b, size_t bytes)
{
	if (b.bytes() >= bytes) return JP_OK;
	HIP_TRY(hipStreamSynchronize(c->stream));
	HIP_TRY(b.reserve(bytes));
	return JP_OK;
}
static int ensure_film(JpContext* c, size_t n_floats) { return reserve_idle(c, c->film, n_floats * sizeof(float)); }

static void free_scene(JpContext* c)
{
	c->tab = SceneTables();
	c->plan.have_scene = false;
	c->plan.pv = PickView(); c->plan.pick = false; c->n_selectable = 0; c->total_weight = 0.0;
	c->plan.tv = TexView(); c->plan.textured = false; c->n_textures = c->n_tex_mats = 0; c->texel_bytes = 0;
	c->side.reset();
}

static int probe_host_sincosf()
{
	static int cached = -1;
	if (cached >= 0) return cached;
	bool okF = true, okN = true;
	uint32_t st = 0x12345u;
	for (int i = 0; i < 200000 && (okF || okN); i++)
	{
		st = st * 1664525u + 1013904223u;
		float y;
		if (i < 150000) y = (float)(st >> 8) * (1.0f / 16777216.0f) * 6.2831855f;
		else if (i < 180000) y = (float)(st >> 8) * (1.0f / 16777216.0f) * 0.01f;
		else y = ((float)(st >> 8) * (1.0f / 16777216.0f) - 0.5f) * 200.f;
		float hs, hc; ::sincosf(y, &hs, &hc);
		const float h1 = ::sinf(y), h2 = ::cosf(y);
		float as, ac, bs, bc;
		jp::sincosf_libm<true>(y, &as, &ac); jp::sincosf_libm<false>(y, &bs, &bc);
		uint32_t uhs, uhc, u1, u2, uas, uac, ubs, ubc;
		std::memcpy(&uhs, &hs, 4); std::memcpy(&uhc, &hc, 4); std::memcpy(&u1, &h1, 4); std::memcpy(&u2, &h2, 4);
		std::memcpy(&uas, &as, 4); std::memcpy(&uac, &ac, 4); std::memcpy(&ubs, &bs, 4); std::memcpy(&ubc, &bc, 4);
		if (uhs != u1 || uhc != u2) { okF = okN = false; }
		if (uas != uhs || uac != uhc) okF = false;
		if (ubs != uhs || ubc != uhc) okN = false;
	}
	cached = okF ? 1 : (okN ? 2 : 0);
	return cached;
}

static int probe_host_libm()
{
	static int cached = -1;
	if (cached >= 0) return cached;
	bool fma_cpu = false;
#if defined(__x86_64__)
	fma_cpu = __builtin_cpu_supports("fma") && __builtin_cpu_supports("avx2");
#endif
	auto same = [](float a, float b) { uint32_t x, y; std::memcpy(&x, &a, 4); std::memcpy(&y, &b, 4); return x == y || (a != a && b != b); };
	auto run = [&](bool fmab) {
		uint32_t st = 0x2545f491u;
		auto rnd = [&]() { st = st * 1664525u + 1013904223u; return st; };
		auto u01 = [&]() { return (float)(rnd() >> 8) * (1.0f / 16777216.0f); };
		for (int i = 0; i < 200000; i++)
		{
			float x, y;
			switch (i & 3)
			{
			case 0: { const uint32_t a = rnd(), b = rnd(); std::memcpy(&x, &a, 4); std::memcpy(&y, &b, 4); break; }
			case 1: x = u01(); y = u01() * 8.f; break;
			case 2: x = (u01() - 0.5f) * 250.f; y = (u01() - 0.5f) * 64.f; break;
			default: x = u01() * 1e-3f; y = 1.f / (u01() * 100.f + 1.f); break;
			}
			const float e = fmab ? jp::lm::expf_libm<true>(x) : jp::lm::expf_libm<false>(x), l = fmab ? jp::lm::logf_libm<true>(x) : jp::lm::logf_libm<false>(x);
			const float pw = fmab ? jp::lm::powf_libm<true>(x, y) : jp::lm::powf_libm<false>(x, y);
			if (!same(e, ::expf(x)) || !same(l, ::logf(x)) || !same(pw, ::powf(x, y))) return false;
			const float a = (i & 3) == 0 ? x : x * 2.f - 1.f;
			if (!same(jp::lm::acosf_libm(a), ::acosf(a)) || !same(jp::lm::atanf_libm(x), ::atanf(x))) return false;
			bool ok; const float t = jp::lm::tanf_libm(x * 8.f, &ok);
			if (ok && !same(t, ::tanf(x * 8.f))) return false;
		}
		return true;
	};
	int mode = 0;
	if (run(fma_cpu)) mode = 1 | (fma_cpu ? 2 : 0);
	else if (run(!fma_cpu)) mode = 1 | (fma_cpu ? 0 : 2);
	cached = mode;
	return cached;
}

static inline unsigned char host_gamma_encoding(float x)
{
	const float c = x < 0.f ? 0.f : (x > 1.f ? 1.f : x);
	return (unsigned char)(std::pow(c, (float)(1 / 2.2)) * 255.0);
}
static const float* host_gamma_thresholds()
{
	static float thr[255]; static std::once_flag once;
	std::call_once(once, []() {
		for (int k = 1; k <= 255; k++)
		{
			uint32_t lo = 0, hi = 0x3f800000u;
			while (hi - lo > 1) { const uint32_t mid = lo + (hi - lo) / 2; float f; std::memcpy(&f, &mid, 4); if (host_gamma_encoding(f) >= k) hi = mid; else lo = mid; }
			std::memcpy(&thr[k - 1], &hi, 4);
		}
	});
	return thr;
}
static unsigned long long host_gamma_sweep(int n_threads)
// ... 118 lines not shown
```

jet-pbrt_amd/csrc/jp_shading.h:

```cpp
#pragma once
#include "jp_device.h"
#define JP_HD_INLINE __host__ __device__ __forceinline__

namespace jp
{
__device__ __forceinline__ void sincos_d(float xf, double* s, double* c)
{
	const double x = (double)xf;
	const double kd = rint(x * 0.63661977236758134308);
	const int k = (int)kd;
	double r = fma(-kd, 1.57079632679489655800e+00, x);
	r = fma(-kd, 6.12323399573676603587e-17, r);
	const double r2 = r * r;
	double sp = fma(r2, -7.6471637318198164759e-13, 1.6059043836821614599e-10);
	sp = fma(sp, r2, -2.5052108385441718775e-08);
	sp = fma(sp, r2, 2.7557319223985890653e-06);
	sp = fma(sp, r2, -1.9841269841269841270e-04);
	sp = fma(sp, r2, 8.3333333333333333333e-03);
	sp = fma(sp, r2, -1.6666666666666666667e-01);
	sp = fma(sp * r2, r, r);
	double cp = fma(r2, 4.7794773323873852974e-14, -1.1470745597729724714e-11);
	cp = fma(cp, r2, 2.0876756987868098979e-09);
	cp = fma(cp, r2, -2.7557319223985890653e-07);
	cp = fma(cp, r2, 2.4801587301587301587e-05);
	cp = fma(cp, r2, -1.3888888888888888889e-03);
	cp = fma(cp, r2, 4.1666666666666666667e-02);
	cp = fma(cp, r2, -0.5);
	cp = fma(cp, r2, 1.0);
	const double ss = (k & 1) ? cp : sp, cc = (k & 1) ? sp : cp;
	*s = (k & 2) ? -ss : ss;
	*c = ((k + 1) & 2) ? -cc : cc;
}

__device__ __constant__ int g_sincosf_mode = 0;

template <bool kFma>
JP_HD_INLINE void sincosf_libm(float y, float* sp, float* cp)
{
	union { float f; unsigned int u; } bits; bits.f = y;
	const unsigned int top = (bits.u >> 20) & 0x7ffu;
	const double x = (double)y;
	double xs, x2; int n = 0;
	if (top <= 0x3f3u)
	{
		if (top <= 0x397u) { *sp = y; *cp = 1.0f; return; }
		xs = x; x2 = x * x;
	}
	else
	{
		const double r = x * 0x1.45f306dc9c883p+23;
		n = ((int)r + 0x800000) >> 24;
		const double xr = kFma ? fma(-(double)n, 0x1.921fb54442d18p+0, x) : x - (double)n * 0x1.921fb54442d18p+0;
		const double sgn = ((n & 3) == 1 || (n & 3) == 2) ? -1.0 : 1.0;
		xs = xr * sgn; x2 = xr * xr;
	}
	const double t = (n & 2) ? -1.0 : 1.0;
	const double c0 = t, c1 = t * -0x1.ffffffd0c621cp-2, c2 = t * 0x1.55553e1068f19p-5, c3 = t * -0x1.6c087e89a359dp-10, c4 = t * 0x1.99343027bf8c3p-16;
	const double s1 = -0x1.555545995a603p-3, s2 = 0x1.1107605230bc4p-7, s3 = -0x1.994eb3774cf24p-13;
	const double x3 = x2 * xs, x4 = x2 * x2;
	const double x5 = x2 * x3, x6 = x2 * x4;
	double c1v, as, ac, bs, bc, S, C;
	if (kFma)
	{
		c1v = fma(x2, c1, c0); as = fma(x2, s3, s2); ac = fma(x2, c4, c3);
		bs = fma(x3, s1, xs); bc = fma(x4, c2, c1v);
		S = fma(as, x5, bs); C = fma(ac, x6, bc);
	}
	else
	{
		c1v = c0 + x2 * c1; as = s2 + x2 * s3; ac = c3 + x2 * c4;
		bs = xs + x3 * s1; bc = c1v + x4 * c2;
		S = bs + x5 * as; C = bc + x6 * ac;
	}
	const float fs = (float)S, fc = (float)C;
	if (n & 1) { *sp = fc; *cp = fs; } else { *sp = fs; *cp = fc; }
}

__device__ __forceinline__ void sincos_f(float xf, float* s, float* c)
{
	const int mode = g_sincosf_mode;
	if (mode == 1 && fabsf(xf) < 120.f) sincosf_libm<true>(xf, s, c);
	else if (mode == 2 && fabsf(xf) < 120.f) sincosf_libm<false>(xf, s, c);
	else { double sd, cd; sincos_d(xf, &sd, &cd); *s = (float)sd; *c = (float)cd; }
}

#define JP_2PI      (2.0f * JP_PI)
#define JP_PI_OVER2 (JP_PI / 2.0f)
#define JP_PI_OVER4 (JP_PI / 4.0f)
#define JP_INV_PI   (1.0f / JP_PI)

enum { BS_REFLECTION = 1, BS_TRANSMISSION = 2, BS_SPECULAR = 4, BS_DIFFUSE = 8, BS_GLOSSY = 16 };
enum { CL_LAMBERT = 0, CL_MIRROR = 1, CL_FRESNEL_SPECULAR = 2, CL_MICROFACET = 3 };
enum { FR_CONDUCTOR = 0, FR_DIELECTRIC = 1 };

struct Frame { V3 s, t, n; };
__device__ __forceinline__ Frame frame_from_z(V3 nn)
{
	Frame f; f.n = normalize(nn);
	V3 tmp = (fabsf(f.n.x) > 0.99f) ? mk(0, 1, 0) : mk(1, 0, 0);
	f.t = normalize(cross(f.n, tmp));
	f.s = normalize(cross(f.t, f.n));
	return f;
}
__device__ __forceinline__ V3 to_local(const Frame& f, V3 w) { return mk(dot(f.s, w), dot(f.t, w), dot(f.n, w)); }
__device__ __forceinline__ V3 to_world(const Frame& f, V3 l) { return f.s * l.x + f.t * l.y + f.n * l.z; }

struct Closure
{
	int kind;
	V3 c0, c1;
	float eta_t;
	float ax, ay;
	int fresnel; V3 feta, fk;
	float lam_o;
};
__device__ __forceinline__ bool is_delta(const Closure& c) { return c.kind == CL_MIRROR || c.kind == CL_FRESNEL_SPECULAR; }

struct BsdfSample { V3 f, wi; float pdf; int flags; };

__device__ __forceinline__ void concentric_disk(float ux, float uy, float& px, float& py)
{
	ux = ux * 2.f - 1.f; uy = uy * 2.f - 1.f;
	if (ux == 0 && uy == 0) { px = 0; py = 0; }
	else
	{
		float radius, theta;
		if (fabsf(ux) > fabsf(uy)) { radius = ux; theta = JP_PI_OVER4 * (uy / ux); }
		else { radius = uy; theta = JP_PI_OVER2 - JP_PI_OVER4 * (ux / uy); }
		float st, ct; sincos_f(theta, &st, &ct);
		px = ct * radius; py = st * radius;
	}
}
__device__ __forceinline__ V3 cosine_hemisphere(float ux, float uy)
{
	float px, py; concentric_disk(ux, uy, px, py);
	float z = sqrtf(smax(0.f, 1 - px * px - py * py));
	return mk(px, py, z);
}
__device__ __forceinline__ V3 uniform_sphere(float ux, float uy)
{
	float z = 1 - 2 * ux;
	float radius = sqrtf(smax(0.f, 1.f - z * z));
	float phi = 2 * JP_PI * uy;
	float sp, cp; sincos_f(phi, &sp, &cp);
	return mk(radius * cp, radius * sp, z);
}

__device__ __forceinline__ bool same_hemi(V3 a, V3 b) { return a.z * b.z > 0; }
__device__ __forceinline__ float sin2t(V3 w) { return smax(0.f, 1.f - w.z * w.z); }
__device__ __forceinline__ float sint(V3 w) { return sqrtf(sin2t(w)); }
__device__ __forceinline__ float tant(V3 w) { return sint(w) / w.z; }
__device__ __forceinline__ float tan2t(V3 w) { return sin2t(w) / (w.z * w.z); }
__device__ __forceinline__ float cosphi(V3 w) { float s = sint(w); return (s == 0) ? 1 : clampf(w.x / s, -1.f, 1.f); }
__device__ __forceinline__ float sinphi(V3 w) { float s = sint(w); return (s == 0) ? 0 : clampf(w.y / s, -1.f, 1.f); }

__device__ __forceinline__ float fresnel_dielectric(float cos_i, float eta_i, float eta_t)
{
	cos_i = clampf(cos_i, -1.f, 1.f);
	bool entering = cos_i > 0.f;
	if (!entering) { float t = eta_i; eta_i = eta_t; eta_t = t; cos_i = fabsf(cos_i); }
	float sin_i = sqrtf(smax(0.f, 1 - cos_i * cos_i));
	float sin_t = eta_i / eta_t * sin_i;
	if (sin_t >= 1) return 1;
	float cos_t = sqrtf(smax(0.f, 1 - sin_t * sin_t));
	float r_para = ((eta_t * cos_i) - (eta_i * cos_t)) / ((eta_t * cos_i) + (eta_i * cos_t));
	float r_perp = ((eta_i * cos_i) - (eta_t * cos_t)) / ((eta_i * cos_i) + (eta_t * cos_t));
	return (r_para * r_para + r_perp * r_perp) / 2;
}

__device__ __forceinline__ V3 fresnel_conductor(float cosI, V3 etai, V3 etat, V3 k)
{
	cosI = clampf(cosI, -1.f, 1.f);
	V3 eta = cdiv(etat, etai), etak = cdiv(k, etai);
	float cos2 = cosI * cosI, sin2 = 1 - cos2;
	V3 eta2 = cmul(eta, eta), etak2 = cmul(etak, etak);
	V3 t0 = eta2 - etak2 - splat(sin2);
	V3 a2plusb2 = csqrt(cmul(t0, t0) + cmul(eta2 * 4.f, etak2));
	V3 t1 = a2plusb2 + splat(cos2);
	V3 a = csqrt((a2plusb2 + t0) * 0.5f);
	V3 t2 = a * (2.f * cosI);
	V3 Rs = cdiv(t1 - t2, t1 + t2);
	V3 t3 = a2plusb2 * cos2 + splat(sin2 * sin2);
	V3 t4 = t2 * sin2;
	V3 Rp = cdiv(cmul(Rs, t3 - t4), t3 + t4);
	return (Rp + Rs) * 0.5f;
}

__device__ __forceinline__ V3 fresnel_eval(const Closure& c, float cosI)
{
	if (c.fresnel == FR_CONDUCTOR) return fresnel_conductor(fabsf(cosI), splat(1.f), c.feta, c.fk);
	return splat(fresnel_dielectric(cosI, 1.5f, 1.f));
}

__device__ __forceinline__ float tr_D(const Closure& c, V3 wh)
{
	float t2 = tan2t(wh);
	if (isinf(t2)) return 0.f;
	const float cos4 = (wh.z * wh.z) * (wh.z * wh.z);
	float cp = cosphi(wh), sp = sinphi(wh);
	float e = (cp * cp / (c.ax * c.ax) + sp * sp / (c.ay * c.ay)) * t2;
	return 1 / (JP_PI * c.ax * c.ay * cos4 * (1 + e) * (1 + e));
}
__device__ __forceinline__ float tr_Lambda(const Closure& c, V3 w)
{
	float absTan = fabsf(tant(w));
	if (isinf(absTan)) return 0.f;
	float cp = cosphi(w), sp = sinphi(w);
	float alpha = sqrtf(cp * cp * c.ax * c.ax + sp * sp * c.ay * c.ay);
	float a2t2 = (alpha * absTan) * (alpha * absTan);
	return (-1 + sqrtf(1.f + a2t2)) / 2;
}
__device__ __forceinline__ void closure_set_wo(Closure& c, V3 wo) { c.lam_o = c.kind == CL_MICROFACET ? tr_Lambda(c, wo) : 0.f; }
__device__ __forceinline__ float tr_G1o(const Closure& c) { return 1 / (1 + c.lam_o); }
__device__ __forceinline__ float tr_G(const Closure& c, V3 wi) { return 1 / (1 + c.lam_o + tr_Lambda(c, wi)); }
__device__ __forceinline__ float tr_Pdf(const Closure& c, V3 wo, V3 wh) { return tr_D(c, wh) * tr_G1o(c) * absdot(wo, wh) / fabsf(wo.z); }

__device__ __forceinline__ void tr_sample11(float cosTheta, float U1, float U2, float* slope_x, float* slope_y)
{
	if ((double)cosTheta > .9999)
	{
		float r = sqrtf(U1 / (1 - U1));
		float phi = 6.28318530718f * U2;
		double sd, cd; sincos_d(phi, &sd, &cd);
		*slope_x = (float)((double)r * cd);
		*slope_y = (float)((double)r * sd);
		return;
	}
	float sinTheta = sqrtf(smax(0.f, 1.f - cosTheta * cosTheta));
	float tanTheta = sinTheta / cosTheta;
	float a = 1 / tanTheta;
	float G1 = 2 / (1 + sqrtf(1.f + 1.f / (a * a)));
	float A = 2 * U1 / G1 - 1;
	float tmp = 1.f / (A * A - 1.f);
	if ((double)tmp > 1e10) tmp = (float)1e10;
	float B = tanTheta;
	float D = sqrtf(smax(B * B * tmp * tmp - (A * A - B * B) * tmp, 0.f));
	float sx1 = B * tmp - D, sx2 = B * tmp + D;
	*slope_x = (A < 0 || sx2 > 1.f / tanTheta) ? sx1 : sx2;
	float S;
	if (U2 > 0.5f) { S = 1.f; U2 = 2.f * (U2 - .5f); }
	else { S = -1.f; U2 = 2.f * (.5f - U2); }
	float z = (U2 * (U2 * (U2 * 0.27385f - 0.73369f) + 0.46341f)) / (U2 * (U2 * (U2 * 0.093073f + 0.309420f) - 1.000000f) + 0.597999f);
	*slope_y = S * z * sqrtf(1.f + *slope_x * *slope_x);
}
__device__ __forceinline__ V3 tr_sample_wh(const Closure& c, V3 wo, float u0, float u1)
{
	bool flip = wo.z < 0;
	V3 wi = flip ? -wo : wo;
	V3 ws = normalize(mk(c.ax * wi.x, c.ay * wi.y, wi.z));
	float sx, sy; tr_sample11(ws.z, u0, u1, &sx, &sy);
	float cp = cosphi(ws), sp = sinphi(ws);
	float tmp = cp * sx - sp * sy;
	sy = sp * sx + cp * sy;
	sx = tmp;
	sx = c.ax * sx; sy = c.ay * sy;
	V3 wh = normalize(mk(-sx, -sy, 1.f));
	if (flip) wh = -wh;
	return wh;
}

__device__ __forceinline__ V3 eval_local(const Closure& c, V3 wo, V3 wi)
{
	if (c.kind == CL_LAMBERT)
	{
		if (!same_hemi(wo, wi)) return splat(0);
		return c.c0 * JP_INV_PI;
	}
	if (c.kind == CL_MICROFACET)
	{
		float cosO = fabsf(wo.z), cosI = fabsf(wi.z);
		V3 wh = wi + wo;
		if (cosI == 0 || cosO == 0) return splat(0);
		if (wh.x == 0 && wh.y == 0 && wh.z == 0) return splat(0);
		wh = normalize(wh);
		V3 ff = (dot(wh, mk(0, 0, 1)) < 0) ? -wh : wh;
		V3 F = fresnel_eval(c, dot(wi, ff));
		return cmul(c.c0 * tr_D(c, wh) * tr_G(c, wi), F) / (4 * cosI * cosO);
	}
	return splat(0);
}

__device__ __forceinline__ BsdfSample sample_local(const Closure& c, V3 wo, float ux, float uy)
{
	BsdfSample s; s.f = splat(0); s.wi = mk(0, 0, 1); s.pdf = 0; s.flags = 0;
	if (c.kind == CL_LAMBERT)
	{
		s.wi = cosine_hemisphere(ux, uy);
		if (wo.z < 0) s.wi.z *= -1;
		s.f = eval_local(c, wo, s.wi);
		s.pdf = same_hemi(wo, s.wi) ? fabsf(s.wi.z) * JP_INV_PI : 0;
		s.flags = BS_REFLECTION | BS_DIFFUSE;
	}
	else if (c.kind == CL_MIRROR)
	{
		s.wi = mk(-wo.x, -wo.y, wo.z);
		s.f = c.c0 / fabsf(s.wi.z);
		s.pdf = 1;
		s.flags = BS_REFLECTION | BS_SPECULAR;
	}
	else if (c.kind == CL_FRESNEL_SPECULAR)
	{
		if (wo.z == 0.f) return s;
		float F = fresnel_dielectric(wo.z, 1.f, c.eta_t);
		if (ux < F)
		{
			s.wi = mk(-wo.x, -wo.y, wo.z);
			s.pdf = F;
			s.f = (c.c0 * F) / fabsf(s.wi.z);
			s.flags = BS_REFLECTION | BS_SPECULAR;
		}
		else
		{
			bool entering = wo.z > 0;
			V3 n = entering ? mk(0, 0, 1) : mk(-0.f, -0.f, -1);
			float etaI = entering ? 1.f : c.eta_t;
			float etaT = entering ? c.eta_t : 1.f;
			float eta = etaI / etaT;
			float cos_i = dot(n, wo);
			float sin2_i = smax(0.f, 1 - cos_i * cos_i);
			float sin2_t = eta * eta * sin2_i;
			if (sin2_t >= 1) { s.f = splat(0); }
			else
			{
				float cos_t = sqrtf(1 - sin2_t);
				s.wi = eta * -wo + (eta * cos_i - cos_t) * n;
				V3 ft = c.c1 * (1 - F);
				ft = ft * ((etaI * etaI) / (etaT * etaT));
				s.pdf = 1 - F;
				s.f = ft / fabsf(s.wi.z);
				s.flags = BS_TRANSMISSION | BS_SPECULAR;
			}
		}
	}
	else
	{
		if (wo.z == 0) return s;
		V3 wh = tr_sample_wh(c, wo, ux, uy);
		float owh = dot(wo, wh);
		if (owh < 0) return s;
		V3 wi = -wo + 2 * owh * wh;
		if (!same_hemi(wo, wi)) return s;
		s.wi = wi;
		s.f = eval_local(c, wo, wi);
		s.pdf = tr_Pdf(c, wo, wh) / (4 * dot(wo, wh));
		s.flags = BS_REFLECTION | BS_GLOSSY;
	}
	return s;
}

template <typename MatPtr>
__device__ __forceinline__ void make_closure(MatPtr mats, int type, int mat, float uplastic, Closure& c)
{
	const float4 p0 = mats[4 * mat + 0], p1 = mats[4 * mat + 1];
	c.c0 = splat(0); c.c1 = splat(0); c.eta_t = 1; c.ax = c.ay = 0; c.fresnel = FR_CONDUCTOR; c.feta = splat(0); c.fk = splat(0);
	if (type == JP_MAT_MATTE) { c.kind = CL_LAMBERT; c.c0 = xyz(p0); }
	else if (type == JP_MAT_MIRROR) { c.kind = CL_MIRROR; c.c0 = xyz(p0); }
	else if (type == JP_MAT_GLASS) { c.kind = CL_FRESNEL_SPECULAR; c.eta_t = p0.x; c.c0 = mk(p0.y, p0.z, p0.w); c.c1 = mk(p1.x, p1.y, p1.z); }
	else if (type == JP_MAT_PLASTIC)
	{
		float Qd = p1.w;
		if (uplastic < Qd) { c.kind = CL_LAMBERT; c.c0 = xyz(p0) / Qd; }
		else { c.kind = CL_MICROFACET; c.c0 = mk(p0.w, p1.x, p1.y) / (1 - Qd); c.fresnel = FR_DIELECTRIC; c.ax = c.ay = smax(0.001f, p1.z); }
	}
	else { c.kind = CL_MICROFACET; c.c0 = splat(1.f); c.fresnel = FR_CONDUCTOR; c.feta = xyz(p0); c.fk = mk(p0.w, p1.x, p1.y); c.ax = smax(0.001f, p1.z); c.ay = smax(0.001f, p1.w); }
}

struct LightSample { V3 pos, wi; float pdf; V3 Li; float dist; };

template <typename PrimPtr, typename LightPtr>
__device__ __forceinline__ LightSample sample_li(const SceneView& sc, PrimPtr prims, LightPtr lights, int li, V3 p, V3 n_isect, float ux, float uy)
{
	LightSample s; s.pos = mk(0, 0, 0); s.wi = mk(0, 0, 0); s.pdf = 0; s.Li = splat(0); s.dist = -1.f;
	const float4 l0 = lights[2 * li], l1 = lights[2 * li + 1];
	const V3 radiance = xyz(l0);
	if (__float_as_int(l0.w) == JP_LIGHT_ENVIRONMENT)
	{
		float theta = uy * JP_PI, phi = ux * 2 * JP_PI;
		float cosT, sinT, sinP, cosP; sincos_f(theta, &sinT, &cosT); sincos_f(phi, &sinP, &cosP);
		s.wi = mk(sinT * cosP, sinT * sinP, cosT);
		s.pos = p + s.wi * 2 * sc.world_radius;
		if (sinT != 0) s.pdf = 1 / (2 * JP_PI * JP_PI * sinT);
		s.Li = radiance;
		return s;
	}
	if (__float_as_int(l0.w) == JP_LIGHT_POINT)
	{
		const V3 wp = xyz(l1);
		s.pos = wp;
		s.wi = normalize(wp - p);
		s.pdf = 1.f;
		s.Li = radiance / len2(wp - p);
		return s;
	}
	if (__float_as_int(l0.w) == JP_LIGHT_DIRECTION)
	{
		s.wi = -xyz(l1);
		s.pos = p + s.wi * 2 * sc.world_radius;
		s.pdf = 1.f;
		s.Li = radiance;
		return s;
	}
	const int pi = __float_as_int(l1.x);
	const float inv_area = l1.y;
	const float4 g0 = prims[4 * pi + 0], g3 = prims[4 * pi + 3];
	const int type = __float_as_int(g3.w);
	V3 lp, ln; float pdf;
	if (type != JP_SHAPE_SPHERE)
	{
		const float4 g1 = prims[4 * pi + 1], g2 = prims[4 * pi + 2];
		if (type == JP_SHAPE_TRIANGLE)
		{
			float su0 = sqrtf(ux); float bx = 1 - su0, by = uy * su0;
			lp = bx * xyz(g0) + by * xyz(g1) + (1 - bx - by) * xyz(g2);
		}
		else if (type == JP_SHAPE_DISK)
		{
			const Frame fr = frame_from_z(xyz(g1));
			float px, py; concentric_disk(ux, uy, px, py);
			lp = xyz(g0) + g0.w * (fr.s * px + fr.t * py);
		}
		else lp = xyz(g1) + (xyz(g0) - xyz(g1)) * ux + (xyz(g2) - xyz(g1)) * uy;
		ln = type == JP_SHAPE_DISK ? xyz(g1) : xyz(g3);
		pdf = inv_area;
		V3 wi = lp - p;
		float dist2 = len2(wi);
		if (dist2 == 0) pdf = 0;
		else
		{
			const float l = sqrtf(dist2);
			wi = wi / l;
			s.dist = l;
			pdf *= dist2 / absdot(ln, -wi);
			if (isinf(pdf)) pdf = 0;
		}
	}
	else
	{
		const V3 c = xyz(g0); const float r = g0.w;
		if (len2(p - c) <= r * r)
		{
			V3 dir = uniform_sphere(ux, uy);
			lp = c + r * dir; ln = normalize(dir);
			pdf = inv_area;
			V3 wi = lp - p;
			if (len2(wi) == 0) pdf = 0;
			else { wi = normalize(wi); pdf *= len2(lp - p) / absdot(n_isect, -wi); }
			if (isinf(pdf)) pdf = 0;
		}
		else
		{
			float dist = len(p - c);
			float inv_dist = 1 / dist;
			float sin_max = r * inv_dist;
			float sin_max2 = sin_max * sin_max;
			float inv_sin_max = 1 / sin_max;
			float cos_max = sqrtf(smax(0.f, 1 - sin_max2));
			float cos_theta = (cos_max - 1) * ux + 1;
			float sin_theta2 = 1 - cos_theta * cos_theta;
			if (sin_max2 < 0.00068523f) { sin_theta2 = sin_max2 * ux; cos_theta = sqrtf(1 - sin_theta2); }
			float cos_alpha = sin_theta2 * inv_sin_max + cos_theta * sqrtf(smax(0.f, 1.f - sin_theta2 * inv_sin_max * inv_sin_max));
			float sin_alpha = sqrtf(smax(0.f, 1.f - cos_alpha * cos_alpha));
			float phi = uy * 2 * JP_PI;
			Frame fr = frame_from_z((c - p) * inv_dist);
			float sphi, cphi; sincos_f(phi, &sphi, &cphi);
			V3 wn = sin_alpha * cphi * (-fr.s) + sin_alpha * sphi * (-fr.t) + cos_alpha * (-fr.n);
			lp = c + r * wn; ln = wn;
			pdf = 1 / (2 * JP_PI * (1 - cos_max));
		}
	}
	s.pos = lp; s.pdf = pdf;
	if (pdf == 0 || len2(lp - p) == 0) s.Li = splat(0);
	else
	{
		s.wi = normalize(lp - p);
		s.Li = (dot(ln, -s.wi) > 0.f) ? radiance : splat(0);
	}
	return s;
}

}
```

jet-pbrt_amd/csrc/jp_upload.h:

```cpp
#pragma once
namespace
{
struct HV3 { float x, y, z; };
inline HV3 hsub(HV3 a, HV3 b) { HV3 r = { a.x - b.x, a.y - b.y, a.z - b.z }; return r; }
inline HV3 hcross(HV3 a, HV3 v) { HV3 r = { a.y * v.z - a.z * v.y, a.z * v.x - a.x * v.z, a.x * v.y - a.y * v.x }; return r; }
inline float hlen(HV3 a) { return std::sqrt(a.x * a.x + a.y * a.y + a.z * a.z); }
inline HV3 hld(const float* p) { HV3 r = { p[0], p[1], p[2] }; return r; }

struct ItemTree { std::vector<int> left, right; std::vector<float> bounds; int height = 0; };
int item_tree_build(const std::vector<float>& ib, std::vector<int>& idx, int start, int end, ItemTree& t, int depth)
{
	const int node = (int)t.left.size(); t.left.push_back(0); t.right.push_back(0); t.bounds.resize(t.bounds.size() + 6);
	t.height = std::max(t.height, depth);
	float nb[6] = { 1e30f, 1e30f, 1e30f, -1e30f, -1e30f, -1e30f }, cb[6] = { 1e30f, 1e30f, 1e30f, -1e30f, -1e30f, -1e30f };
	for (int i = start; i < end; i++)
	{
		const float* b = &ib[6 * (size_t)idx[i]];
		for (int a = 0; a < 3; a++) { nb[a] = std::min(nb[a], b[a]); nb[3 + a] = std::max(nb[3 + a], b[3 + a]); const float c = 0.5f * (b[a] + b[3 + a]); cb[a] = std::min(cb[a], c); cb[3 + a] = std::max(cb[3 + a], c); }
	}
	std::memcpy(&t.bounds[6 * (size_t)node], nb, sizeof(nb));
	if (end - start == 1) { t.left[node] = -idx[start] - 1; return node; }
	auto area = [](const float* b) { const float dx = b[3] - b[0], dy = b[4] - b[1], dz = b[5] - b[2]; return (dx < 0 || dy < 0 || dz < 0) ? 0.f : dx * dy + dy * dz + dz * dx; };
	const int NB = 16; float bestCost = 3.0e38f; int bestAxis = -1, bestBin = -1;
	for (int a = 0; a < 3; a++)
// ... 477 lines not shown
		const bool want_wide = opt_flag(op.device_wide, s->n_primitives > 64);
		if (want_wide)
		{
			WideResult wr;
			e = lbvh_build_wide(c->stream, c->tab.nodes.get<float4>(), s->n_primitives, wr);
			if (e != hipSuccess) return fail(JP_ERR_DEVICE, std::string("jp_upload_scene: device wide-tree build failed: ") + hipGetErrorString(e));
			if (wr.wide) { c->tab.wide = std::move(wr.wide); dev_wide = true; dev_n_wide = wr.n_wide; wide_height = wr.height; use_wide = true; c->build_ms += wr.build_ms; }
		}
		const bool want_q4 = s->n_primitives > 1024 && opt_flag(op.q4, true);
		if (want_q4)
		{
			WideResult qr;
			e = lbvh_build_q4(c->stream, c->tab.nodes.get<float4>(), s->n_primitives, qr);
			if (e != hipSuccess) return fail(JP_ERR_DEVICE, std::string("jp_upload_scene: device 4-wide tree build failed: ") + hipGetErrorString(e));
			if (qr.wide) { c->tab.q4 = std::move(qr.wide); dev_q4 = true; dev_n_q4 = qr.n_wide; c->build_ms += qr.build_ms; use_q4 = true; q4_height = qr.height; }
		}
	}
	c->bvh_height = height; c->bvh_nodes = ref_sem ? s->n_bvh_nodes : (int)(n4nodes / 4);

	std::vector<float4> flat;
	if (!device_build && !ref_sem && s->n_primitives <= 64)
	{
		int nleaves = 0; for (int n = 0; n < s->n_bvh_nodes; n++) if (seen[n] && s->bvh_left[n] < 0) nleaves++;
		if (nleaves <= 32)
		{
			for (int n = 0; n < s->n_bvh_nodes; n++)
			{
				if (!seen[n] || s->bvh_left[n] >= 0) continue;
				float bb[6]; pad_box(n, bb);
				int first = -s->bvh_left[n] - 1, cnt = s->bvh_right[n];
				unsigned long long bits = 0;
				for (int k = 0; k < cnt; k++) bits |= 1ull << devPrimOf[s->bvh_prim_index[first + k]];
				const uint32_t lo = (uint32_t)bits, hi = (uint32_t)(bits >> 32); float flo, fhi; std::memcpy(&flo, &lo, 4); std::memcpy(&fhi, &hi, 4);
				flat.push_back(make_float4(bb[0], bb[1], bb[2], flo)); flat.push_back(make_float4(bb[3], bb[4], bb[5], fhi));
			}
		}
	}

	std::vector<float4> mats(4 * std::max(1, s->n_materials)); std::vector<int> mtype(std::max(1, s->n_materials), 0);
	for (int i = 0; i < s->n_materials; i++) { std::memcpy(&mats[4 * i], s->mat_params + (size_t)i * JP_MAT_PARAM_STRIDE, 16 * sizeof(float)); mtype[i] = s->mat_type[i]; }
	std::vector<float4> lights(2 * std::max(1, s->n_lights)); int planes = 0, nenv = 0; float envsum[3] = { 0, 0, 0 };
	std::vector<float> light_area(pick ? (size_t)s->n_lights : 0, 0.f);
	for (int i = 0; i < s->n_lights; i++)
	{
		int ty = s->light_type[i]; float tf; std::memcpy(&tf, &ty, 4);
		const float* rad = s->light_radiance + 3 * i;
		lights[2 * i] = make_float4(rad[0], rad[1], rad[2], tf);
		bool black = rad[0] == 0.f && rad[1] == 0.f && rad[2] == 0.f;
		if (!black) planes++;
		float inv_area = 0.f; int dp = -1;
		if (ty == JP_LIGHT_AREA)
		{
			int p = s->light_prim[i]; dp = devPrimOf[p];
			int t = s->prim_shape_type[p], k = s->prim_shape_index[p]; float area;
			if (t == JP_SHAPE_TRIANGLE) area = 0.5f * hlen(hcross(hsub(hld(s->tri_p1 + 3 * k), hld(s->tri_p0 + 3 * k)), hsub(hld(s->tri_p2 + 3 * k), hld(s->tri_p0 + 3 * k))));
			else if (t == JP_SHAPE_RECTANGLE) area = hlen(hcross(hsub(hld(s->rect_p0 + 3 * k), hld(s->rect_p1 + 3 * k)), hsub(hld(s->rect_p2 + 3 * k), hld(s->rect_p1 + 3 * k))));
			else if (t == JP_SHAPE_DISK) { const float kPi = (float)3.14159265358979323846; area = kPi * s->disk_radius[k] * s->disk_radius[k]; }
			else { const float kPi = (float)3.14159265358979323846; float r2 = s->sph_radius[k] * s->sph_radius[k]; area = 4 * kPi * r2; }
			inv_area = 1 / area;
			if (pick) light_area[i] = area;
		}
		else if (ty == JP_LIGHT_ENVIRONMENT) { nenv++; envsum[0] += rad[0]; envsum[1] += rad[1]; envsum[2] += rad[2]; }
		float df; std::memcpy(&df, &dp, 4);
		lights[2 * i + 1] = make_float4(df, inv_area, 0, 0);
		if (ty == JP_LIGHT_POINT || ty == JP_LIGHT_DIRECTION) lights[2 * i + 1] = make_float4(s->light_vec[3 * i], s->light_vec[3 * i + 1], s->light_vec[3 * i + 2], 0);
	}

	SceneTables& T = c->tab;
	if (!device_build)
	{
		HIP_TRY(upload(T.nodes, nodes.data(), nodes.size() * sizeof(float4)));
		HIP_TRY(upload(T.prims, prims.data(), prims.size() * sizeof(float4)));
		HIP_TRY(upload(T.meta, meta.data(), meta.size() * sizeof(int4)));
	}
	HIP_TRY(upload(T.mats, mats.data(), mats.size() * sizeof(float4)));
	HIP_TRY(upload(T.mat_type, mtype.data(), mtype.size() * sizeof(int)));
	HIP_TRY(upload(T.lights, lights.data(), lights.size() * sizeof(float4)));
	{
		std::vector<float4> tabv;
		if (!pick) tabv.insert(tabv.end(), lights.begin(), lights.begin() + 2 * (size_t)s->n_lights);
		tabv.insert(tabv.end(), mats.begin(), mats.begin() + 4 * (size_t)s->n_materials);
		const size_t at = tabv.size(); tabv.resize(at + ((size_t)s->n_materials + 3) / 4, make_float4(0, 0, 0, 0));
		if (s->n_materials > 0) std::memcpy(&tabv[at], mtype.data(), (size_t)s->n_materials * sizeof(int));
		if (!device_build)
		{
			tabv.insert(tabv.end(), prims.begin(), prims.end());
			const size_t am = tabv.size(); tabv.resize(am + meta.size());
			std::memcpy(&tabv[am], meta.data(), meta.size() * sizeof(int4));
			auto hnorm = [](HV3 a) { const float l = hlen(a); HV3 r = { a.x / l, a.y / l, a.z / l }; return r; };
			for (size_t pi = 0; pi < meta.size(); pi++)
			{
				const float4 g3 = prims[4 * pi + 3], g1 = prims[4 * pi + 1];
				int type; std::memcpy(&type, &g3.w, 4);
				const HV3 nn = type == JP_SHAPE_DISK ? HV3{ g1.x, g1.y, g1.z } : HV3{ g3.x, g3.y, g3.z };
				const HV3 n = hnorm(nn);
				const HV3 tmp = std::fabs(n.x) > 0.99f ? HV3{ 0, 1, 0 } : HV3{ 1, 0, 0 };
				const HV3 t = hnorm(hcross(n, tmp)), sv = hnorm(hcross(t, n));
				tabv.push_back(make_float4(n.x, n.y, n.z, 0)); tabv.push_back(make_float4(sv.x, sv.y, sv.z, 0)); tabv.push_back(make_float4(t.x, t.y, t.z, 0));
			}
		}
		HIP_TRY(upload(T.shade_tab, tabv.data(), tabv.size() * sizeof(float4)));
	}
	if (use_wide && !dev_wide) HIP_TRY(upload(T.wide, wide.data(), wide.size() * sizeof(uint32_t)));
	if ((use_q4 && !dev_q4) || use_cert) HIP_TRY(upload(T.q4, q4.data(), q4.size() * sizeof(uint32_t)));
	if (use_cert) HIP_TRY(upload(T.refbox, refbox.data(), refbox.size() * sizeof(float4)));
	if (!flat.empty()) HIP_TRY(upload(T.flat, flat.data(), flat.size() * sizeof(float4)));

	ScenePlan& p = c->plan; SceneView& v = p.sv;
	v.nodes = T.nodes.get<float4>(); v.n_nodes = (int)(n4nodes / 4);
	v.prims = T.prims.get<float4>(); v.meta = T.meta.get<int4>(); v.n_prims = (int)nmeta;
	v.mats = T.mats.get<float4>(); v.mat_type = T.mat_type.get<int>(); v.n_mats = s->n_materials;
	v.lights = T.lights.get<float4>(); v.n_lights = s->n_lights; v.shade_tab = T.shade_tab.get<float4>();
	v.env_sum = make_float3(envsum[0], envsum[1], envsum[2]); v.n_env = nenv;
	v.world_radius = s->world_radius; v.cam = s->camera;
	v.flat = T.flat.get<float4>(); v.n_flat = (int)(flat.size() / 2);
	v.wide = T.wide.get<uint4>(); v.n_wide = dev_wide ? dev_n_wide : (int)(wide.size() / 20);
	v.q4 = T.q4.get<uint4>(); v.n_q4 = dev_q4 ? dev_n_q4 : (int)(q4.size() / 16);
	v.refbox = T.refbox.get<float4>(); v.cert_pad = cert_pad; v.cert_pad_eye = cert_pad_eye; p.cert = use_cert;
	p.use_q4 = use_q4; p.q4_shadow = use_q4 && opt_flag(op.q4_shadow, true);
	p.stack_depth = std::max(2, height + 2);
	p.stack_depth_q4 = (use_q4 || use_cert) ? 3 * q4_height + 2 : 0;
	size_t scene_bytes = (n4nodes + n4prims) / 4 * 5 * sizeof(float4);
	size_t prim_bytes = n4prims / 4 * 5 * sizeof(float4);
	size_t stack_bytes = (size_t)p.stack_depth * JP_BLOCK * sizeof(int);
	p.scene_in_lds = !device_build && scene_bytes + stack_bytes <= 40 * 1024;
	p.trav_mode = use_wide ? 3 : ((!flat.empty() && prim_bytes <= 40 * 1024) ? 2 : (p.scene_in_lds ? 1 : 0));
	if (!use_wide && op.traversal > 0) { const int m = op.traversal - 1; if (m == 0 || (m == 1 && p.scene_in_lds)) p.trav_mode = m; }
	if (use_wide) p.scene_in_lds = false;
	if (ref_sem) p.trav_mode = 5;
	p.lds_bytes = p.trav_mode == 2 ? prim_bytes : (p.trav_mode == 1 ? stack_bytes + scene_bytes : stack_bytes);
	p.lds_bytes_shadow = p.trav_mode == 3 ? (size_t)2 * (wide_height + 2) * JP_BLOCK * sizeof(int) : p.lds_bytes;
	{
		if (pick) planes = std::min(planes, 1);
		size_t tab = ((pick ? (size_t)0 : (size_t)2 * s->n_lights) + (size_t)4 * s->n_materials) * sizeof(float4) + (size_t)s->n_materials * sizeof(int) + 16;
		p.tables_in_lds = tab <= 16 * 1024;
		const size_t shade_static = (size_t)JP_SHADE_TILE * 3 + (size_t)JP_SHADE_CLASSES * (JP_SHADE_TILE / JP_BLOCK) * (JP_BLOCK / 64) * 4 + 128;
		const size_t prim_part = n4prims * sizeof(float4) + nmeta * sizeof(int4) + 3 * nmeta * sizeof(float4);
		p.shade_prims_in_lds = p.tables_in_lds && p.scene_in_lds && tab + prim_part <= 24 * 1024;
		p.shade_lds_bytes = p.tables_in_lds ? tab + (p.shade_prims_in_lds ? prim_part : 0) : 0;
		const size_t stage_bytes = 16 + (size_t)std::max(1, planes) * 2 * JP_BLOCK * sizeof(float4);
		p.stage_nee = p.tables_in_lds && std::max(1, planes) <= 4 && shade_static + p.shade_lds_bytes + stage_bytes <= 64 * 1024;
		if (p.stage_nee) p.shade_lds_bytes += stage_bytes;
	}
	p.n_planes = std::max(1, planes);
	{
		bool kinds[8] = { false, false, false, false, false, false, false, false }; int nk = 0;
		for (int i = 0; i < s->n_primitives; i++) { const int m = s->prim_material[i]; const int k = m < 0 ? 7 : s->mat_type[m]; if (!kinds[k]) { kinds[k] = true; nk++; } }
		p.stack_lds_words = op.stack_lds_words >= 2 ? (op.stack_lds_words & ~1) : 12;
		p.persist = ((p.trav_mode == 0 || p.trav_mode == 3 || p.trav_mode == 5) && s->n_primitives > 1024) ? 16 : 0;
		if (op.persist != 0) p.persist = op.persist < 0 ? 0 : op.persist;
		p.vote = opt_flag(op.vote, p.trav_mode != 5 || p.cert);
		p.class_mask = 1; for (int k = 0; k < 5; k++) if (kinds[k]) p.class_mask |= 2 << k;
		p.shade_sort = opt_flag(op.shade_sort, nk > 1);
	}
	p.has_null_material = hasNull; c->cert_fell_back = false;
	if (pick) { const int st = upload_light_table(c, s, light_area); if (st != JP_OK) { free_scene(c); return st; } }
	p.have_scene = true;
	return JP_OK;
}


extern "C" int jp_upload_scene_textured(JpContext* c, const JpScene* s, const JpTextures* t)
{
	if (!c || !s) return fail(JP_ERR_INVALID_ARGUMENT, "jp_upload_scene_textured: null argument");
	if (!t) return jp_upload_scene(c, s);
	if (t->struct_bytes < (int32_t)sizeof(JpTextures)) return fail(JP_ERR_INVALID_ARGUMENT, "jp_upload_scene_textured: JpTextures.struct_bytes smaller than this library's JpTextures");
	if (t->n_textures < 0 || t->n_textures > (1 << 28)) return fail(JP_ERR_INVALID_ARGUMENT, "jp_upload_scene_textured: n_textures out of range");
	if (t->n_textures == 0) return jp_upload_scene(c, s);
	const int nt = t->n_textures;
	if (!t->tex_type || !t->tex_color) return fail(JP_ERR_INVALID_ARGUMENT, "jp_upload_scene_textured: null tex_type / tex_color");
	if (t->n_materials != s->n_materials) return fail(JP_ERR_INVALID_ARGUMENT, "jp_upload_scene_textured: n_materials differs from the scene's");
	if (t->n_triangles != s->n_triangles) return fail(JP_ERR_INVALID_ARGUMENT, "jp_upload_scene_textured: n_triangles differs from the scene's");
	if (t->n_materials > 0 && (!t->mat_texture || !s->mat_type)) return fail(JP_ERR_INVALID_ARGUMENT, "jp_upload_scene_textured: null mat_texture");
	long long pool = 0;
	for (int i = 0; i < nt; i++)
	{
		const int ty = t->tex_type[i];
		if (ty < JP_TEXTURE_SOLID || ty > JP_TEXTURE_IMAGE) return fail(JP_ERR_INVALID_ARGUMENT, "jp_upload_scene_textured: unknown texture type");
		if (ty == JP_TEXTURE_IMAGE)
		{
			if (!t->tex_width || !t->tex_height || !t->tex_offset || !t->texels) return fail(JP_ERR_INVALID_ARGUMENT, "jp_upload_scene_textured: image texture without tex_width / tex_height / tex_offset / texels");
			const long long w = t->tex_width[i], h = t->tex_height[i], off = t->tex_offset[i];
			if (w < 1 || w > 16384 || h < 1 || h > 16384) return fail(JP_ERR_INVALID_ARGUMENT, "jp_upload_scene_textured: image size out of range (1 .. 16384 per side)");
			if (off < 0 || t->n_texel_bytes < 0 || off > t->n_texel_bytes - 3 * w * h) return fail(JP_ERR_INVALID_ARGUMENT, "jp_upload_scene_textured: image texels beyond n_texel_bytes");
			pool += w * h;
		}
		else
		{
			const int nc = ty == JP_TEXTURE_CHECKER ? 6 : 3;
			for (int k = 0; k < nc; k++) if (!std::isfinite(t->tex_color[6 * (size_t)i + k])) return fail(JP_ERR_INVALID_ARGUMENT, "jp_upload_scene_textured: colour not finite");
		}
	}
	if (pool > 0x7fffffffll) return fail(JP_ERR_INVALID_ARGUMENT, "jp_upload_scene_textured: more than 2^31 texels in all");
	int ntm = 0;
	for (int m = 0; m < t->n_materials; m++)
	{
		const int k = t->mat_texture[m];
		if (k < -1 || k >= nt) return fail(JP_ERR_INVALID_ARGUMENT, "jp_upload_scene_textured: mat_texture out of range");
		if (k < 0) continue;
		const int mt = s->mat_type[m];
		if (mt != JP_MAT_MATTE && mt != JP_MAT_MIRROR && mt != JP_MAT_PLASTIC) return fail(JP_ERR_INVALID_ARGUMENT, "jp_upload_scene_textured: a texture on a glass or metal material (its [0..2] is eta, not a colour)");
		ntm++;
	}
	if (s->n_primitives > 0 && (!s->prim_shape_type || !s->prim_shape_index)) return fail(JP_ERR_INVALID_ARGUMENT, "jp_upload_scene_textured: null array");
	const int st = jp_upload_scene(c, s);
	if (st != JP_OK) return st;
	if (ntm == 0) return JP_OK;

	std::vector<int4> desc(nt); std::vector<float4> col(2 * (size_t)nt); std::vector<unsigned int> texels((size_t)pool);
	size_t at = 0;
	for (int i = 0; i < nt; i++)
	{
		const float* cc = t->tex_color + 6 * (size_t)i;
		desc[i] = make_int4(t->tex_type[i], 0, 0, 0);
		col[2 * i] = make_float4(0, 0, 0, 0); col[2 * i + 1] = make_float4(0, 0, 0, 0);
		if (t->tex_type[i] == JP_TEXTURE_IMAGE)
		{
			const int w = t->tex_width[i], h = t->tex_height[i];
			desc[i].y = w; desc[i].z = h; desc[i].w = (int)at;
			const uint8_t* src = t->texels + t->tex_offset[i];
			for (size_t k = 0; k < (size_t)w * h; k++) texels[at + k] = (unsigned int)src[3 * k] | ((unsigned int)src[3 * k + 1] << 8) | ((unsigned int)src[3 * k + 2] << 16) | 0xff000000u;
			at += (size_t)w * h;
		}
		else
		{
			col[2 * i] = make_float4(cc[0], cc[1], cc[2], 0);
			if (t->tex_type[i] == JP_TEXTURE_CHECKER) col[2 * i + 1] = make_float4(cc[3], cc[4], cc[5], 0);
		}
	}
	std::vector<int> mt(t->mat_texture, t->mat_texture + t->n_materials);
	std::vector<float2> puv(3 * (size_t)s->n_primitives, make_float2(0, 0));
	if (t->tri_uv)
		for (int p = 0; p < s->n_primitives; p++)
			if (s->prim_shape_type[p] == JP_SHAPE_TRIANGLE)
			{
				const float* u = t->tri_uv + 6 * (size_t)s->prim_shape_index[p];
				for (int k = 0; k < 3; k++) puv[3 * (size_t)p + k] = make_float2(u[2 * k], u[2 * k + 1]);
			}
	SceneTables& T = c->tab;
	if (upload(T.tex_desc, desc.data(), desc.size() * sizeof(int4)) != hipSuccess || upload(T.tex_col, col.data(), col.size() * sizeof(float4)) != hipSuccess
	    || upload(T.texels, texels.data(), texels.size() * sizeof(unsigned int)) != hipSuccess || upload(T.mat_tex, mt.data(), mt.size() * sizeof(int)) != hipSuccess
	    || upload(T.prim_uv, puv.data(), puv.size() * sizeof(float2)) != hipSuccess)
	{
		free_scene(c);
		return fail(JP_ERR_DEVICE, "jp_upload_scene_textured: out of device memory for the texture tables");
	}
	TexView& tv = c->plan.tv; tv = TexView();
	tv.desc = T.tex_desc.get<int4>(); tv.col = T.tex_col.get<float4>(); tv.texels = T.texels.get<unsigned int>();
	tv.mat_tex = T.mat_tex.get<int>(); tv.prim_uv = T.prim_uv.get<float2>();
	c->plan.textured = true; c->n_textures = nt; c->n_tex_mats = ntm; c->texel_bytes = (long long)texels.size() * 4;
	return JP_OK;
}
```

Baseline: 2988.

## Specialize extend, shadow and shade kernels for flat-shape, area-light, non-delta scenes

Adds a compile-time feature trait that strips sphere/disk intersection, non-area light sampling and delta/plastic material branches from traversal and shading code. At upload the host records which shape types, light types and light shapes the scene uses, and picks the lean kernel instantiations when the scene qualifies (flat traversal mode, prims and NEE staged in LDS). The aim is less branch divergence, fewer registers and smaller code on simple scenes like the Cornell box. The cost is more template instantiations and a code path that is only correct when the scene masks are accurate.

Result: faster. 3134, median of 6 (+4.9%).

```diff
diff --git a/jet-pbrt_amd/csrc/jp_device.h b/jet-pbrt_amd/csrc/jp_device.h
--- a/jet-pbrt_amd/csrc/jp_device.h
+++ b/jet-pbrt_amd/csrc/jp_device.h
@@ -56,6 +56,12 @@
 	const float4* refbox; float cert_pad, cert_pad_eye;
 };
 
+template <bool kCurved, bool kOtherLights, bool kDelta>
+struct Feat { static constexpr bool curved = kCurved, other_lights = kOtherLights, delta = kDelta; };
+typedef Feat<true, true, true> FeatAll;
+typedef Feat<false, true, true> FeatFlat;
+typedef Feat<false, false, false> FeatLean;
+
 __device__ __forceinline__ bool tri_hit(V3 p0, V3 p1, V3 p2, V3 n, V3 o, V3 d, float tmin, float& tmax)
 {
 	const V3 oa = p0 - o;
@@ -117,14 +123,17 @@
 	return false;
 }
 
-template <int kS, typename PrimPtr>
+template <int kS, typename F = FeatAll, typename PrimPtr>
 __device__ __forceinline__ bool prim_hit(PrimPtr prims, int pi, V3 o, V3 d, float tmin, float& tmax)
 {
 	const float4 g0 = prims[kS * pi + 0], g1 = prims[kS * pi + 1], g2 = prims[kS * pi + 2], g3 = prims[kS * pi + 3];
 	const int type = __float_as_int(g3.w);
 	if (type == JP_SHAPE_TRIANGLE) return tri_hit(xyz(g0), xyz(g1), xyz(g2), xyz(g3), o, d, tmin, tmax);
-	if (type == JP_SHAPE_SPHERE) return sph_hit(xyz(g0), g0.w, o, d, tmin, tmax);
-	if (type == JP_SHAPE_DISK) return disk_hit(xyz(g0), g0.w, xyz(g1), o, d, tmin, tmax);
+	if constexpr (F::curved)
+	{
+		if (type == JP_SHAPE_SPHERE) return sph_hit(xyz(g0), g0.w, o, d, tmin, tmax);
+		if (type == JP_SHAPE_DISK) return disk_hit(xyz(g0), g0.w, xyz(g1), o, d, tmin, tmax);
+	}
 	return rect_hit(xyz(g0), xyz(g1), xyz(g2), mk(g0.w, g1.w, g2.w), xyz(g3), o, d, tmin, tmax);
 }
 
@@ -263,7 +272,7 @@
 	return mask;
 }
 
-template <bool kAnyHit, bool k64, int kS, typename PrimPtr>
+template <bool kAnyHit, bool k64, int kS, typename F = FeatAll, typename PrimPtr>
 __device__ __forceinline__ int flat_prims(typename FlatMask<k64>::type mask, PrimPtr prims, V3 o, V3 d, float tmin, float& tmax)
 {
 	int hit = -1;
@@ -274,16 +283,16 @@
 	{
 		const int p = (k64 ? __ffsll((unsigned long long)mask) : __ffs((int)mask)) - 1;
 		mask &= mask - 1;
-		if (prim_hit<kS>(prims, p, o, d, tmin, tmax)) { hit = p; if (kAnyHit) return hit; }
+		if (prim_hit<kS, F>(prims, p, o, d, tmin, tmax)) { hit = p; if (kAnyHit) return hit; }
 	}
 	return hit;
 }
 
-template <bool kAnyHit, int kS, typename PrimPtr>
+template <bool kAnyHit, int kS, typename F = FeatAll, typename PrimPtr>
 __device__ __forceinline__ int traverse_flat(const float4* flat_g, int n_flat, int n_prims, PrimPtr prims, V3 o, V3 d, float tmin, float& tmax)
 {
-	if (n_prims > 32) return flat_prims<kAnyHit, true, kS>(flat_boxes<true>(flat_g, n_flat, o, d, tmin, tmax), prims, o, d, tmin, tmax);
-	return flat_prims<kAnyHit, false, kS>(flat_boxes<false>(flat_g, n_flat, o, d, tmin, tmax), prims, o, d, tmin, tmax);
+	if (n_prims > 32) return flat_prims<kAnyHit, true, kS, F>(flat_boxes<true>(flat_g, n_flat, o, d, tmin, tmax), prims, o, d, tmin, tmax);
+	return flat_prims<kAnyHit, false, kS, F>(flat_boxes<false>(flat_g, n_flat, o, d, tmin, tmax), prims, o, d, tmin, tmax);
 }
 
 template <bool kAnyHit, typename PrimPtr>
diff --git a/jet-pbrt_amd/csrc/jp_kernels.hip b/jet-pbrt_amd/csrc/jp_kernels.hip
--- a/jet-pbrt_amd/csrc/jp_kernels.hip
+++ b/jet-pbrt_amd/csrc/jp_kernels.hip
@@ -66,7 +66,7 @@
 #else
 #define JP_TT(i) do { } while (0)
 #endif
-template <int kMode>
+template <int kMode, typename F = FeatAll>
 struct SceneAccess;
 template <> struct SceneAccess<0>
 {
@@ -90,7 +90,7 @@
 	template <bool kAnyHit> __device__ __forceinline__ int trace(const SceneView&, V3 o, V3 d, float tmin, float& tmax) const
 	{ return traverse<kAnyHit, 5>(nodes, prims, o, d, tmin, tmax, stack); }
 };
-template <> struct SceneAccess<2>
+template <typename F> struct SceneAccess<2, F>
 {
 	float4* prims;
 	__device__ __forceinline__ SceneAccess(const SceneView& sc, int)
@@ -100,7 +100,7 @@
 		__syncthreads();
 	}
 	template <bool kAnyHit> __device__ __forceinline__ int trace(const SceneView& sc, V3 o, V3 d, float tmin, float& tmax) const
-	{ return traverse_flat<kAnyHit, 5>(sc.flat, sc.n_flat, sc.n_prims, prims, o, d, tmin, tmax); }
+	{ return traverse_flat<kAnyHit, 5, F>(sc.flat, sc.n_flat, sc.n_prims, prims, o, d, tmin, tmax); }
 };
 
 template <> struct SceneAccess<3>
@@ -135,10 +135,10 @@
 	{ return traverse_ref<kAnyHit>(nodes, prims, o, d, tmin, tmax, stack); }
 };
 
-template <int kMode>
+template <int kMode, typename F = FeatAll>
 __global__ void __launch_bounds__(JP_BLOCK) k_extend(SceneView sc, Queues q, int cur, int depth, DevCounters* cnt)
 {
-	SceneAccess<kMode> acc(sc, depth);
+	SceneAccess<kMode, F> acc(sc, depth);
 	const unsigned int b = blockIdx.x, n = q.blk_q[cur][b], rbase = b * q.R;
 	if (b == 0 && threadIdx.x == 0) { cnt->closest += cnt->n_queue[cur]; cnt->n_queue[cur ^ 1] = 0; cnt->n_shadow = 0; }
 	unsigned int h = 0;
@@ -161,7 +161,7 @@
 #ifndef JP_SHADE_TILE
 #define JP_SHADE_TILE 8192
 #endif
-template <bool kTab, bool kPrims, bool kStage, bool kSort, bool kTex, bool kPick>
+template <bool kTab, bool kPrims, bool kStage, bool kSort, bool kTex, bool kPick, typename F = FeatAll>
 __device__ __forceinline__ void shade_body(SceneView sc, Queues q, RenderConst rc, int cur, DevCounters* cnt, const TexView& tv, const PickView& pv)
 {
 	static_assert(kTab || !kPrims, "k_shade: primitive records in LDS only together with the tables");
@@ -333,7 +333,7 @@
 				const int type = __float_as_int(g3.w);
 				p = o + h.x * d;
 				if (type == JP_SHAPE_TRIANGLE) N = xyz(g3);
-				else if (type == JP_SHAPE_RECTANGLE) { nflip = !(dot(xyz(g3), d) <= 0); N = nflip ? -xyz(g3) : xyz(g3); }
+				else if (!F::curved || type == JP_SHAPE_RECTANGLE) { nflip = !(dot(xyz(g3), d) <= 0); N = nflip ? -xyz(g3) : xyz(g3); }
 				else if (type == JP_SHAPE_DISK) N = xyz(prims[4 * pi + 1]);
 				else { const float4 g0 = prims[4 * pi]; N = normalize(p - xyz(g0)); tabframe = false; }
 				hitprim = pi;
@@ -344,7 +344,7 @@
 					if (dot(N, wo) > 0.f) Le = xyz(lights[2 * meta.z]);
 				}
 			}
-			else if (bounce == 0 || spec)
+			else if (F::other_lights && (bounce == 0 || spec))
 			{
 				if (kPick)
 				{
@@ -379,13 +379,13 @@
 				{
 					float up = 0.f;
 					const int mtype = mat_type[mat];
-					if (mtype == JP_MAT_PLASTIC) up = rngf(rc, key, dim++);
+					if (F::delta && mtype == JP_MAT_PLASTIC) up = rngf(rc, key, dim++);
 					if (kTex && sw != 0u) make_closure_tex(mats, mtype, mat, up, tex_color(tv, sw), c);
-					else make_closure(mats, mtype, mat, up, c);
+					else make_closure<F>(mats, mtype, mat, up, c);
 #ifdef JP_DBG_SKIP_FRAME
 					fr.n = N; fr.s = mk(N.y, N.z, N.x); fr.t = mk(N.z, N.x, N.y);
 #else
-					if (kPrims && tabframe)
+					if (kPrims && (!F::curved || tabframe))
 					{
 						const float4 fn = s_frames[3 * hitprim], fs = s_frames[3 * hitprim + 1], ft = s_frames[3 * hitprim + 2];
 						fr.n = nflip ? -xyz(fn) : xyz(fn); fr.s = xyz(fs); fr.t = nflip ? -xyz(ft) : xyz(ft);
@@ -393,7 +393,7 @@
 					else fr = frame_from_z(N);
 #endif
 					shaded = true;
-					wantNee = !is_delta(c);
+					wantNee = !is_delta<F>(c);
 #ifdef JP_DBG_SKIP_NEE
 					wantNee = false;
 #endif
@@ -431,12 +431,12 @@
 					const float4 lrad = lights[2 * li];
 					if (isblack(xyz(lrad))) continue;
 					const float ux = rngf(rc, key, d0), uy = rngf(rc, key, d0 + 1);
-					LightSample ls = sample_li(sc, prims, lights, li, p, N, ux, uy);
+					LightSample ls = sample_li<F>(sc, prims, lights, li, p, N, ux, uy);
 					if (isblack(ls.Li) || ls.pdf == 0.f) continue;
-					const V3 f = eval_local(c, wo, to_local(fr, ls.wi));
+					const V3 f = eval_local<F>(c, wo, to_local(fr, ls.wi));
 					if (isblack(f)) continue;
-					const V3 sdir = __float_as_int(lrad.w) == JP_LIGHT_AREA ? ls.wi : normalize(ls.pos - p);
-					const float dist = ls.dist >= 0.f ? ls.dist : len(p - ls.pos);
+					const V3 sdir = (!F::other_lights || __float_as_int(lrad.w) == JP_LIGHT_AREA) ? ls.wi : normalize(ls.pos - p);
+					const float dist = (!F::other_lights || ls.dist >= 0.f) ? ls.dist : len(p - ls.pos);
 					V3 contrib = cmul(cmul(beta, f), ls.Li) * absdot(ls.wi, N) / ls.pdf;
 					if (kPick) contrib = contrib / pmf;
 					if (k < rc.n_planes)
@@ -465,7 +465,7 @@
 #endif
 		{
 			const float ux = rngf(rc, key, dim), uy = rngf(rc, key, dim + 1); dim += 2;
-			BsdfSample bs = sample_local(c, wo, ux, uy);
+			BsdfSample bs = sample_local<F>(c, wo, ux, uy);
 			bs.wi = to_world(fr, bs.wi);
 			if (!(isblack(bs.f) || bs.pdf == 0.f))
 			{
@@ -539,20 +539,20 @@
 		if (run_sh) atomicAdd(&cnt->n_shadow, run_sh);
 	}
 }
-template <bool kTab, bool kPrims, bool kStage, bool kSort>
+template <bool kTab, bool kPrims, bool kStage, bool kSort, typename F = FeatAll>
 __global__ void __launch_bounds__(JP_BLOCK) k_shade(SceneView sc, Queues q, RenderConst rc, int cur, DevCounters* cnt)
 {
 	const TexView tv = {}; const PickView pv = {};
-	shade_body<kTab, kPrims, kStage, kSort, false, false>(sc, q, rc, cur, cnt, tv, pv);
-}
-
-template <int kMode>
+	shade_body<kTab, kPrims, kStage, kSort, false, false, F>(sc, q, rc, cur, cnt, tv, pv);
+}
+
+template <int kMode, typename F = FeatAll>
 __global__ void __launch_bounds__(JP_BLOCK, 4) k_shadow(SceneView sc, Queues q, RenderConst rc, int depth, DevCounters* cnt)
 {
 #ifdef JP_TRAV_TIMING
 	unsigned long long t_acc[10] = { 0, 0, 0, 0, 0, 0, 0, 0, 0, 0 }, t_last = __builtin_amdgcn_s_memtime();
 #endif
-	SceneAccess<kMode> acc(sc, depth);
+	SceneAccess<kMode, F> acc(sc, depth);
 	const unsigned int b = blockIdx.x, E = q.blk_sh[b], rbase = b * q.R;
 	JP_TT(0);
 	unsigned int rays = 0, occ = 0;
@@ -587,7 +587,7 @@
 			{
 				const unsigned int m = flat_boxes<false>(sc.flat, sc.n_flat, xyz(so), dir, 0.001f, tmax);
 				JP_TT(4);
-				hit = flat_prims<true, false, 5>(m, acc.prims, xyz(so), dir, 0.001f, tmax);
+				hit = flat_prims<true, false, 5, F>(m, acc.prims, xyz(so), dir, 0.001f, tmax);
 				JP_TT(5);
 			}
 			else hit = acc.template trace<true>(sc, xyz(so), dir, 0.001f, tmax);
diff --git a/jet-pbrt_amd/csrc/jp_render.h b/jet-pbrt_amd/csrc/jp_render.h
--- a/jet-pbrt_amd/csrc/jp_render.h
+++ b/jet-pbrt_amd/csrc/jp_render.h
@@ -75,6 +75,15 @@
 inline int deepest_walk(const ScenePlan& p) { return std::max(std::max(p.stack_depth, p.stack_depth_q4), p.trav_mode == 3 ? (int)(p.lds_bytes_shadow / (JP_BLOCK * sizeof(int))) : 0); }
 inline size_t spill_need(const ScenePlan& p, int deep, unsigned int G) { return deep >= p.stack_lds_words ? (size_t)(deep - p.stack_lds_words + 1) * G * JP_BLOCK : 1; }
 
+inline bool flat_shapes_only(int shape_mask) { return (shape_mask & ~((1 << JP_SHAPE_TRIANGLE) | (1 << JP_SHAPE_RECTANGLE))) == 0; }
+inline bool lean_traversal(const ScenePlan& p, bool generic) { return !generic && p.trav_mode == 2 && flat_shapes_only(p.shape_mask); }
+inline bool lean_shading(const ScenePlan& p, bool generic)
+{
+	const int delta_classes = (2 << JP_MAT_MIRROR) | (2 << JP_MAT_GLASS) | (2 << JP_MAT_PLASTIC);
+	return !generic && p.shade_prims_in_lds && p.stage_nee && flat_shapes_only(p.shape_mask) && (p.light_mask & ~(1 << JP_LIGHT_AREA)) == 0
+	    && flat_shapes_only(p.light_shape_mask) && (p.class_mask & delta_classes) == 0;
+}
+
 typedef void (*ExtendKernel)(SceneView, Queues, int, int, DevCounters*);
 typedef void (*ExtendRefillKernel)(SceneView, Queues, int, int, int*, DevCounters*);
 struct ExtendLaunch { ExtendRefillKernel refill; ExtendKernel plain; size_t lds; int words; };
@@ -83,8 +92,9 @@
 	static const ExtendRefillKernel k[3][2] = { { k_extend_persist<M, 8, false>, k_extend_persist<M, 8, true> }, { k_extend_persist<M, 16, false>, k_extend_persist<M, 16, true> }, { k_extend_persist<M, 32, false>, k_extend_persist<M, 32, true> } };
 	return k[refill_row(p)][p.vote];
 }
-ExtendLaunch extend_kernel(const ScenePlan& p)
-{
+ExtendLaunch extend_kernel(const ScenePlan& p, bool generic)
+{
+	if (lean_traversal(p, generic)) return { nullptr, k_extend<2, FeatFlat>, p.lds_bytes, p.stack_depth };
 	if (!refill_walks(p)) return { nullptr, p.trav_mode == 5 ? k_extend<5> : (p.trav_mode == 2 ? k_extend<2> : (p.trav_mode == 1 ? k_extend<1> : k_extend<0>)), p.lds_bytes, p.stack_depth };
 	const int words = std::min(extend_depth(p), p.stack_lds_words);
 	const ExtendRefillKernel k = p.trav_mode == 5 ? (p.cert ? extend_refill<6>(p) : extend_refill<5>(p)) : (p.use_q4 ? extend_refill<4>(p) : extend_refill<0>(p));
@@ -99,10 +109,11 @@
 	static const ShadowRefillKernel k[3][2] = { { k_shadow_persist<M, 8, false>, k_shadow_persist<M, 8, true> }, { k_shadow_persist<M, 16, false>, k_shadow_persist<M, 16, true> }, { k_shadow_persist<M, 32, false>, k_shadow_persist<M, 32, true> } };
 	return k[refill_row(p)][p.vote];
 }
-ShadowLaunch shadow_kernel(const ScenePlan& p, unsigned int R)
+ShadowLaunch shadow_kernel(const ScenePlan& p, unsigned int R, bool generic)
 {
 	const int words = std::min(shadow_depth(p), p.stack_lds_words);
 	const size_t plds = (size_t)words * JP_BLOCK * sizeof(int) + (((size_t)R * p.n_planes + 31) / 32) * 4 * (p.cert ? 2 : 1);
+	if (lean_traversal(p, generic)) return { nullptr, k_shadow<2, FeatFlat>, p.lds_bytes, p.stack_depth, p.cert };
 	if (!refill_walks(p) || plds > 64 * 1024)
 		return { nullptr, p.trav_mode == 3 ? k_shadow<3> : (p.trav_mode == 5 ? k_shadow<5> : (p.trav_mode == 2 ? k_shadow<2> : (p.trav_mode == 1 ? k_shadow<1> : k_shadow<0>))), p.trav_mode == 3 ? p.lds_bytes_shadow : p.lds_bytes, p.stack_depth, p.cert };
 	const ShadowRefillKernel k = p.trav_mode == 5 ? (p.cert ? shadow_refill<6>(p) : shadow_refill<5>(p)) : (p.q4_shadow ? shadow_refill<4>(p) : (p.trav_mode == 3 ? shadow_refill<3>(p) : shadow_refill<0>(p)));
@@ -117,8 +128,14 @@
 	ShadeKernels k = { sort ? k_shade<kTab, kPrims, kStage, true> : k_shade<kTab, kPrims, kStage, false>, sort ? k_shade_tex<kTab, kPrims, kStage, true> : k_shade_tex<kTab, kPrims, kStage, false> };
 	return k;
 }
-ShadeKernels shade_kernels(const ScenePlan& p)
-{
+ShadeKernels shade_kernels(const ScenePlan& p, bool generic)
+{
+	if (lean_shading(p, generic))
+	{
+		ShadeKernels k = shade_row<true, true, true>(p.shade_sort);
+		k.plain = p.shade_sort ? k_shade<true, true, true, true, FeatLean> : k_shade<true, true, true, false, FeatLean>;
+		return k;
+	}
 	if (p.shade_prims_in_lds) return p.stage_nee ? shade_row<true, true, true>(p.shade_sort) : shade_row<true, true, false>(p.shade_sort);
 	if (p.tables_in_lds) return p.stage_nee ? shade_row<true, false, true>(p.shade_sort) : shade_row<true, false, false>(p.shade_sort);
 	return shade_row<false, false, false>(p.shade_sort);
@@ -205,7 +222,8 @@
 		rc.compact = (p.trav_mode != 2 && p.trav_mode != 1 && npix % JP_BLOCK == 0) ? 1 : 0;
 		if (c->opt.compact_regions != 0) rc.compact = (c->opt.compact_regions > 0 && npix % JP_BLOCK == 0) ? 1 : 0;
 		const int grid = (int)G;
-		const ExtendLaunch ek = extend_kernel(p); const ShadowLaunch sk = shadow_kernel(p, R); const ShadeKernels hk = shade_kernels(p); const OtherKernel ok = other_kernel(p);
+		const bool generic = c->opt.reserved[0] == 1;
+		const ExtendLaunch ek = extend_kernel(p, generic); const ShadowLaunch sk = shadow_kernel(p, R, generic); const ShadeKernels hk = shade_kernels(p, generic); const OtherKernel ok = other_kernel(p);
 		const ShadePickKernels pk = p.pick ? shade_pick_kernels(p) : ShadePickKernels{ nullptr, nullptr };
 		for (int s0 = 0; s0 < rp->spp; s0 += sbatch)
 		{
diff --git a/jet-pbrt_amd/csrc/jp_runtime.h b/jet-pbrt_amd/csrc/jp_runtime.h
--- a/jet-pbrt_amd/csrc/jp_runtime.h
+++ b/jet-pbrt_amd/csrc/jp_runtime.h
@@ -50,6 +50,7 @@
 	int n_planes = 1; bool has_null_material = false;
 	bool tables_in_lds = false, stage_nee = false; size_t shade_lds_bytes = 0;
 	int class_mask = 0x3f; bool shade_sort = false;
+	int shape_mask = 0xf, light_mask = 0xf, light_shape_mask = 0xf;
 	int stack_lds_words = 12;
 };
 
diff --git a/jet-pbrt_amd/csrc/jp_shading.h b/jet-pbrt_amd/csrc/jp_shading.h
--- a/jet-pbrt_amd/csrc/jp_shading.h
+++ b/jet-pbrt_amd/csrc/jp_shading.h
@@ -114,7 +114,8 @@
 	int fresnel; V3 feta, fk;
 	float lam_o;
 };
-__device__ __forceinline__ bool is_delta(const Closure& c) { return c.kind == CL_MIRROR || c.kind == CL_FRESNEL_SPECULAR; }
+template <typename F = FeatAll>
+__device__ __forceinline__ bool is_delta(const Closure& c) { if constexpr (!F::delta) return false; else return c.kind == CL_MIRROR || c.kind == CL_FRESNEL_SPECULAR; }
 
 struct BsdfSample { V3 f, wi; float pdf; int flags; };
 
@@ -186,9 +187,10 @@
 	return (Rp + Rs) * 0.5f;
 }
 
+template <typename F = FeatAll>
 __device__ __forceinline__ V3 fresnel_eval(const Closure& c, float cosI)
 {
-	if (c.fresnel == FR_CONDUCTOR) return fresnel_conductor(fabsf(cosI), splat(1.f), c.feta, c.fk);
+	if (!F::delta || c.fresnel == FR_CONDUCTOR) return fresnel_conductor(fabsf(cosI), splat(1.f), c.feta, c.fk);
 	return splat(fresnel_dielectric(cosI, 1.5f, 1.f));
 }
 
@@ -259,6 +261,7 @@
 	return wh;
 }
 
+template <typename F = FeatAll>
 __device__ __forceinline__ V3 eval_local(const Closure& c, V3 wo, V3 wi)
 {
 	if (c.kind == CL_LAMBERT)
@@ -266,7 +269,7 @@
 		if (!same_hemi(wo, wi)) return splat(0);
 		return c.c0 * JP_INV_PI;
 	}
-	if (c.kind == CL_MICROFACET)
+	if (!F::delta || c.kind == CL_MICROFACET)
 	{
 		float cosO = fabsf(wo.z), cosI = fabsf(wi.z);
 		V3 wh = wi + wo;
@@ -274,12 +277,13 @@
 		if (wh.x == 0 && wh.y == 0 && wh.z == 0) return splat(0);
 		wh = normalize(wh);
 		V3 ff = (dot(wh, mk(0, 0, 1)) < 0) ? -wh : wh;
-		V3 F = fresnel_eval(c, dot(wi, ff));
-		return cmul(c.c0 * tr_D(c, wh) * tr_G(c, wi), F) / (4 * cosI * cosO);
+		V3 Fr = fresnel_eval<F>(c, dot(wi, ff));
+		return cmul(c.c0 * tr_D(c, wh) * tr_G(c, wi), Fr) / (4 * cosI * cosO);
 	}
 	return splat(0);
 }
 
+template <typename FS = FeatAll>
 __device__ __forceinline__ BsdfSample sample_local(const Closure& c, V3 wo, float ux, float uy)
 {
 	BsdfSample s; s.f = splat(0); s.wi = mk(0, 0, 1); s.pdf = 0; s.flags = 0;
@@ -287,18 +291,18 @@
 	{
 		s.wi = cosine_hemisphere(ux, uy);
 		if (wo.z < 0) s.wi.z *= -1;
-		s.f = eval_local(c, wo, s.wi);
+		s.f = eval_local<FS>(c, wo, s.wi);
 		s.pdf = same_hemi(wo, s.wi) ? fabsf(s.wi.z) * JP_INV_PI : 0;
 		s.flags = BS_REFLECTION | BS_DIFFUSE;
 	}
-	else if (c.kind == CL_MIRROR)
+	else if (FS::delta && c.kind == CL_MIRROR)
 	{
 		s.wi = mk(-wo.x, -wo.y, wo.z);
 		s.f = c.c0 / fabsf(s.wi.z);
 		s.pdf = 1;
 		s.flags = BS_REFLECTION | BS_SPECULAR;
 	}
-	else if (c.kind == CL_FRESNEL_SPECULAR)
+	else if (FS::delta && c.kind == CL_FRESNEL_SPECULAR)
 	{
 		if (wo.z == 0.f) return s;
 		float F = fresnel_dielectric(wo.z, 1.f, c.eta_t);
@@ -341,22 +345,22 @@
 		V3 wi = -wo + 2 * owh * wh;
 		if (!same_hemi(wo, wi)) return s;
 		s.wi = wi;
-		s.f = eval_local(c, wo, wi);
+		s.f = eval_local<FS>(c, wo, wi);
 		s.pdf = tr_Pdf(c, wo, wh) / (4 * dot(wo, wh));
 		s.flags = BS_REFLECTION | BS_GLOSSY;
 	}
 	return s;
 }
 
-template <typename MatPtr>
+template <typename F = FeatAll, typename MatPtr>
 __device__ __forceinline__ void make_closure(MatPtr mats, int type, int mat, float uplastic, Closure& c)
 {
 	const float4 p0 = mats[4 * mat + 0], p1 = mats[4 * mat + 1];
 	c.c0 = splat(0); c.c1 = splat(0); c.eta_t = 1; c.ax = c.ay = 0; c.fresnel = FR_CONDUCTOR; c.feta = splat(0); c.fk = splat(0);
 	if (type == JP_MAT_MATTE) { c.kind = CL_LAMBERT; c.c0 = xyz(p0); }
-	else if (type == JP_MAT_MIRROR) { c.kind = CL_MIRROR; c.c0 = xyz(p0); }
-	else if (type == JP_MAT_GLASS) { c.kind = CL_FRESNEL_SPECULAR; c.eta_t = p0.x; c.c0 = mk(p0.y, p0.z, p0.w); c.c1 = mk(p1.x, p1.y, p1.z); }
-	else if (type == JP_MAT_PLASTIC)
+	else if (F::delta && type == JP_MAT_MIRROR) { c.kind = CL_MIRROR; c.c0 = xyz(p0); }
+	else if (F::delta && type == JP_MAT_GLASS) { c.kind = CL_FRESNEL_SPECULAR; c.eta_t = p0.x; c.c0 = mk(p0.y, p0.z, p0.w); c.c1 = mk(p1.x, p1.y, p1.z); }
+	else if (F::delta && type == JP_MAT_PLASTIC)
 	{
 		float Qd = p1.w;
 		if (uplastic < Qd) { c.kind = CL_LAMBERT; c.c0 = xyz(p0) / Qd; }
@@ -367,13 +371,13 @@
 
 struct LightSample { V3 pos, wi; float pdf; V3 Li; float dist; };
 
-template <typename PrimPtr, typename LightPtr>
+template <typename F = FeatAll, typename PrimPtr, typename LightPtr>
 __device__ __forceinline__ LightSample sample_li(const SceneView& sc, PrimPtr prims, LightPtr lights, int li, V3 p, V3 n_isect, float ux, float uy)
 {
 	LightSample s; s.pos = mk(0, 0, 0); s.wi = mk(0, 0, 0); s.pdf = 0; s.Li = splat(0); s.dist = -1.f;
 	const float4 l0 = lights[2 * li], l1 = lights[2 * li + 1];
 	const V3 radiance = xyz(l0);
-	if (__float_as_int(l0.w) == JP_LIGHT_ENVIRONMENT)
+	if (F::other_lights && __float_as_int(l0.w) == JP_LIGHT_ENVIRONMENT)
 	{
 		float theta = uy * JP_PI, phi = ux * 2 * JP_PI;
 		float cosT, sinT, sinP, cosP; sincos_f(theta, &sinT, &cosT); sincos_f(phi, &sinP, &cosP);
@@ -383,7 +387,7 @@
 		s.Li = radiance;
 		return s;
 	}
-	if (__float_as_int(l0.w) == JP_LIGHT_POINT)
+	if (F::other_lights && __float_as_int(l0.w) == JP_LIGHT_POINT)
 	{
 		const V3 wp = xyz(l1);
 		s.pos = wp;
@@ -392,7 +396,7 @@
 		s.Li = radiance / len2(wp - p);
 		return s;
 	}
-	if (__float_as_int(l0.w) == JP_LIGHT_DIRECTION)
+	if (F::other_lights && __float_as_int(l0.w) == JP_LIGHT_DIRECTION)
 	{
 		s.wi = -xyz(l1);
 		s.pos = p + s.wi * 2 * sc.world_radius;
@@ -405,7 +409,7 @@
 	const float4 g0 = prims[4 * pi + 0], g3 = prims[4 * pi + 3];
 	const int type = __float_as_int(g3.w);
 	V3 lp, ln; float pdf;
-	if (type != JP_SHAPE_SPHERE)
+	if (!F::other_lights || type != JP_SHAPE_SPHERE)
 	{
 		const float4 g1 = prims[4 * pi + 1], g2 = prims[4 * pi + 2];
 		if (type == JP_SHAPE_TRIANGLE)
@@ -413,14 +417,14 @@
 			float su0 = sqrtf(ux); float bx = 1 - su0, by = uy * su0;
 			lp = bx * xyz(g0) + by * xyz(g1) + (1 - bx - by) * xyz(g2);
 		}
-		else if (type == JP_SHAPE_DISK)
+		else if (F::other_lights && type == JP_SHAPE_DISK)
 		{
 			const Frame fr = frame_from_z(xyz(g1));
 			float px, py; concentric_disk(ux, uy, px, py);
 			lp = xyz(g0) + g0.w * (fr.s * px + fr.t * py);
 		}
 		else lp = xyz(g1) + (xyz(g0) - xyz(g1)) * ux + (xyz(g2) - xyz(g1)) * uy;
-		ln = type == JP_SHAPE_DISK ? xyz(g1) : xyz(g3);
+		ln = (F::other_lights && type == JP_SHAPE_DISK) ? xyz(g1) : xyz(g3);
 		pdf = inv_area;
 		V3 wi = lp - p;
 		float dist2 = len2(wi);
diff --git a/jet-pbrt_amd/csrc/jp_upload.h b/jet-pbrt_amd/csrc/jp_upload.h
--- a/jet-pbrt_amd/csrc/jp_upload.h
+++ b/jet-pbrt_amd/csrc/jp_upload.h
@@ -653,6 +653,15 @@
 		p.vote = opt_flag(op.vote, p.trav_mode != 5 || p.cert);
 		p.class_mask = 1; for (int k = 0; k < 5; k++) if (kinds[k]) p.class_mask |= 2 << k;
 		p.shade_sort = opt_flag(op.shade_sort, nk > 1);
+		p.shape_mask = 0; p.light_mask = 0; p.light_shape_mask = 0;
+		for (int i = 0; i < s->n_primitives; i++) p.shape_mask |= 1 << (s->prim_shape_type[i] & 3);
+		for (int i = 0; i < s->n_lights; i++)
+		{
+			const float* rad = s->light_radiance + 3 * i;
+			if (rad[0] == 0.f && rad[1] == 0.f && rad[2] == 0.f) continue;
+			p.light_mask |= 1 << (s->light_type[i] & 3);
+			if (s->light_type[i] == JP_LIGHT_AREA) p.light_shape_mask |= 1 << (s->prim_shape_type[s->light_prim[i]] & 3);
+		}
 	}
 	p.has_null_material = hasNull; c->cert_fell_back = false;
 	if (pick) { const int st = upload_light_table(c, s, light_area); if (st != JP_OK) { free_scene(c); return st; } }
```
